# drprojects/superpoint_transformer

Hardware: AMD Instinct MI355X
Metric: Mpoints/s SPT fwd+bwd on S3DIS-scale NAG (higher is better)
Workload: dtype f32 (the reference's shipped matmul class - configs/train.yaml:60-61 `float32_matmul_precision: high` = TF32 / bf16x3 next to `precision: 32` - as bf16x3: matrix products on the bf16 pipe with split operands, attention and the backward of the fused layers and of the attention blocks' Linears hi*hi +

## Files before the change

include/spt_hip.h:

```cpp
#ifndef SPT_HIP_H
#define SPT_HIP_H

#include <stddef.h>
#include <stdint.h>

#ifdef __cplusplus
extern "C" {
#endif

typedef void* spt_stream_t;

enum spt_reduce_op {
  SPT_SUM = 0,
  SPT_MEAN = 1,
  SPT_MIN = 2,
  SPT_MAX = 3
};

typedef struct spt_gn_fwd_tables {
  const float* weight;
  const float* mean_scale;
  float eps;
  float* mean;
  float* rstd;
// ... 462 lines not shown
size_t spt_fused_linear_workspace_bytes(int K, int N);
int spt_fused_linear_fwd_f32(const float* x, int64_t r0, int64_t r1, int K, const float* W,
                             int N, const float* pre_am, const float* pre_scale,
                             const float* pre_bias, float pre_slope, float* h, double* total,
                             void* ws, size_t ws_bytes, spt_stream_t stream);
int spt_fused_linear_bwd_f32(const float* gy, const float* h, int64_t r0, int64_t r1, int N,
                             const float* am, const float* scale, const float* bias,
                             float slope, const float* c1, const float* c2, const float* c3,
                             const float* xprev, int K, const float* pre_am,
                             const float* pre_scale, const float* pre_bias, float pre_slope,
                             const float* W, float* gx, float* gW, int accumulate,
                             double* prev_total, void* ws, size_t ws_bytes, spt_stream_t stream);
int spt_fused_linear_pooled_supported(int K, int N);
int spt_fused_linear_pooled_supported_ex(int K, int N, int mode);
#define SPT_FMLP_BWD_REGISTER_STAGED 4
#define SPT_FMLP_H_BF16 8
#define SPT_FMLP_X_BF16 16
int spt_fused_linear_storage_supported(int K, int N);
int spt_fused_linear_bwd_use_dma(int on);
int spt_fused_linear_bwd_route(int K0, int K, int N, int mode);
int spt_fused_linear_fwd_use_x3(int on);
int spt_fused_linear_fwd_ex_f32(const float* x, int64_t r0, int64_t r1, int K, const float* W,
                                int N, const float* pre_am, const float* pre_scale,
                                const float* pre_bias, float pre_slope, float* h, double* total,
                                int mode, void* ws, size_t ws_bytes, spt_stream_t stream);
int spt_fused_linear_bwd_ex_f32(const float* gy, const float* h, int64_t r0, int64_t r1, int N,
                                const float* am, const float* scale, const float* bias,
                                float slope, const float* c1, const float* c2, const float* c3,
                                const float* xprev, int K, const float* pre_am,
                                const float* pre_scale, const float* pre_bias, float pre_slope,
                                const float* W, float* gx, float* gW, int accumulate,
                                double* prev_total, int mode, void* ws, size_t ws_bytes,
                                spt_stream_t stream);
int spt_fused_linear_bwd_pooled_ex_f32(
    const float* gout, const int32_t* arg, const int32_t* perm, const int32_t* pos_seg,
    const float* h, int64_t p0, int64_t p1, int N, const float* am, const float* scale,
    const float* bias, float slope, const float* c1, const float* c2, const float* c3,
    const float* xprev, int K, const float* pre_am, const float* pre_scale, const float* pre_bias,
    float pre_slope, const float* W, float* gx, float* gW, int accumulate, double* prev_total,
    int mode, void* ws, size_t ws_bytes, spt_stream_t stream);
int spt_fused_linear_bwd_pooled_f32(
    const float* gout, const int32_t* arg, const int32_t* perm, const int32_t* pos_seg,
    const float* h, int64_t p0, int64_t p1, int N, const float* am, const float* scale,
    const float* bias, float slope, const float* c1, const float* c2, const float* c3,
    const float* xprev, int K, const float* pre_am, const float* pre_scale, const float* pre_bias,
    float pre_slope, const float* W, float* gx, float* gW, int accumulate, double* prev_total,
    void* ws, size_t ws_bytes, spt_stream_t stream);

int spt_fused_linear_fwd_runs_f32(const float* x, int nruns, const int64_t* run_r0,
                                  const int64_t* run_r1, const int32_t* run_graph, int num_graphs,
                                  int K, const float* W, int N, const float* pre_am,
                                  const float* pre_scale, const float* pre_bias, float pre_slope,
                                  float* h, double* total, int mode, void* ws, size_t ws_bytes,
                                  spt_stream_t stream);
int spt_fused_linear_bwd_runs_f32(
    const float* gy, const float* h, int nruns, const int64_t* run_r0, const int64_t* run_r1,
    const int32_t* run_graph, int num_graphs, int N, const float* am, const float* scale,
    const float* bias, float slope, const float* c1, const float* c2, const float* c3,
    const float* xprev, int K, const float* pre_am, const float* pre_scale, const float* pre_bias,
    float pre_slope, const float* W, float* gx, float* gW, double* prev_total, int mode, void* ws,
    size_t ws_bytes, spt_stream_t stream);
int spt_fused_linear_bwd_pooled_runs_f32(
    const float* gout, const int32_t* arg, const int32_t* perm, const int32_t* pos_seg,
    const float* h, int nruns, const int64_t* run_p0, const int64_t* run_p1,
    const int32_t* run_graph, int num_graphs, int N, const float* am, const float* scale,
    const float* bias, float slope, const float* c1, const float* c2, const float* c3,
    const float* xprev, int K, const float* pre_am, const float* pre_scale, const float* pre_bias,
    float pre_slope, const float* W, float* gx, float* gW, double* prev_total, int mode, void* ws,
    size_t ws_bytes, spt_stream_t stream);
int spt_fused_linear_fwd_runs_gn_f32(const float* x, int nruns, const int64_t* run_r0,
                                     const int64_t* run_r1, const int32_t* run_graph, int num_graphs,
                                     int K, const float* W, int N, const float* pre_am,
                                     const float* pre_scale, const float* pre_bias, float pre_slope,
                                     float* h, double* total, int mode, void* ws, size_t ws_bytes,
                                     const spt_gn_fwd_tables* norm, spt_stream_t stream);
int spt_fused_linear_bwd_runs_gn_f32(
    const float* gy, const float* h, int nruns, const int64_t* run_r0, const int64_t* run_r1,
    const int32_t* run_graph, int num_graphs, int N, const float* am, const float* scale,
    const float* bias, float slope, const float* c1, const float* c2, const float* c3,
    const float* xprev, int K, const float* pre_am, const float* pre_scale, const float* pre_bias,
    float pre_slope, const float* W, float* gx, float* gW, double* prev_total, int mode, void* ws,
    size_t ws_bytes, const spt_gn_bwd_tables* prev_norm, spt_stream_t stream);
int spt_fused_linear_bwd_fold_supported(int K0, int K, int N, int mode);
int spt_fused_linear_bwd_runs_gn_fold_f32(
    const float* gy, const float* h, int nruns, const int64_t* run_r0, const int64_t* run_r1,
    const int32_t* run_graph, int num_graphs, int N, const float* am, const float* scale,
    const float* bias, float slope, const float* c1, const float* c2, const float* c3,
    const float* xprev, int K, const float* pre_am, const float* pre_scale, const float* pre_bias,
    float pre_slope, const float* W, float* gW, int mode, void* ws, size_t ws_bytes,
    const spt_gn_bwd_tables* prev_norm, const float* x0, int K0, const float* W0, float* gW0,
    spt_stream_t stream);
int spt_fused_linear_bwd_pooled_runs_gn_f32(
    const float* gout, const int32_t* arg, const int32_t* perm, const int32_t* pos_seg,
    const float* h, int nruns, const int64_t* run_p0, const int64_t* run_p1,
    const int32_t* run_graph, int num_graphs, int N, const float* am, const float* scale,
    const float* bias, float slope, const float* c1, const float* c2, const float* c3,
    const float* xprev, int K, const float* pre_am, const float* pre_scale, const float* pre_bias,
    float pre_slope, const float* W, float* gx, float* gW, double* prev_total, int mode, void* ws,
    size_t ws_bytes, const spt_gn_bwd_tables* prev_norm, spt_stream_t stream);

int spt_csr_check_i64(const int64_t* idx, const int64_t* points, const int64_t* pointers, int64_t n,
                      int64_t num_seg, int check_ascending, int32_t* flag, spt_stream_t stream);
int spt_csr_adopt_i64(const int64_t* idx, const int64_t* points, const int64_t* pointers, int64_t n,
                      int64_t num_seg, int32_t* perm32, int32_t* rowptr32, int32_t* flag,
                      spt_stream_t stream);

int spt_fused_linear_pool_supported(int K, int N, int mode);
size_t spt_fused_linear_pool_gram_len(int K);
size_t spt_fused_linear_pool_workspace_bytes(int K, int N);
int spt_fused_linear_fwd_pool_runs_f32(
    const void* x, const int32_t* perm, const int32_t* pos_seg, const int32_t* rowptr,
    const int64_t* seg_graph, int64_t num_seg, int64_t n_rows, int nruns, const int64_t* run_p0,
    const int64_t* run_p1, const int32_t* run_graph, int num_graphs, int K, const float* W, int N,
    const float* gn_weight, const float* gn_bias, const float* gn_mean_scale, float eps, float slope,
    const float* pre_am, const float* pre_scale, const float* pre_bias, float pre_slope, float* out,
    int32_t* arg, int32_t* argpos, float* raw, double* gram, double* total, float* mean, float* rstd,
    float* am, float* scale, int mode, void* ws, size_t ws_bytes, spt_stream_t stream);
int spt_fused_linear_bwd_pool_runs_f32(
    const float* gout, const float* raw, const int32_t* argpos, const int32_t* perm,
    const int32_t* pos_seg, const int64_t* seg_graph, int64_t num_seg, int nruns,
    const int64_t* run_p0, const int64_t* run_p1, const int32_t* run_graph, int num_graphs, int N,
    const float* am, const float* scale, const float* bias, float slope, const float* c1,
    const float* c2, const float* c3, const void* xprev, int K, const float* pre_am,
    const float* pre_scale, const float* pre_bias, float pre_slope, const float* W,
    const double* gram, float* gm, float* gx, float* gW, double* prev_total, int mode, void* ws,
    size_t ws_bytes, spt_stream_t stream);
int spt_fused_linear_bwd_pool_runs_gn_f32(
    const float* gout, const float* raw, const int32_t* argpos, const int32_t* perm,
    const int32_t* pos_seg, const int64_t* seg_graph, int64_t num_seg, int nruns,
    const int64_t* run_p0, const int64_t* run_p1, const int32_t* run_graph, int num_graphs, int N,
    const float* am, const float* scale, const float* bias, float slope, const float* c1,
    const float* c2, const float* c3, const void* xprev, int K, const float* pre_am,
    const float* pre_scale, const float* pre_bias, float pre_slope, const float* W,
    const double* gram, float* gm, float* gx, float* gW, double* prev_total, int mode, void* ws,
    size_t ws_bytes, const spt_gn_bwd_tables* prev_norm, spt_stream_t stream);

size_t spt_cross_entropy_workspace_bytes(int64_t rows);
int spt_cross_entropy_fwd_f32(const float* logits, const int64_t* target, int64_t rows, int C,
                              int64_t ignore_index, float* lse, float* loss, float* count,
                              void* ws, size_t ws_bytes, spt_stream_t stream);
int spt_cross_entropy_bwd_f32(const float* logits, const int64_t* target, const float* lse,
                              int64_t rows, int C, int64_t ignore_index, const float* gout,
                              const float* count, float* glogits, spt_stream_t stream);

int spt_hist_loss_fwd_f32(const float* logits, const int64_t* target, int64_t rows, int C, int ncols,
                          int mode, int64_t ignore_index, const float* weight, float* loss,
                          double* den, int64_t* confmat, void* ws, size_t ws_bytes,
                          spt_stream_t stream);
int spt_hist_loss_bwd_f32(const float* logits, const int64_t* target, int64_t rows, int C, int ncols,
                          int mode, int64_t ignore_index, const float* weight, const float* gout,
                          const double* den, float* glogits, spt_stream_t stream);
size_t spt_edge_affinity_loss_workspace_bytes(int64_t E);
int spt_edge_affinity_loss_fwd_f32(const float* logits, const float* target,
                                   const int64_t* edge_index, int64_t E, const uint8_t* node_void,
                                   const int64_t* node_obj, const int64_t* node_y, int64_t N,
                                   const float* case_weight, const float* pos_weight, float* loss,
                                   double* den, int64_t* stats, int32_t* status, void* ws,
                                   size_t ws_bytes, spt_stream_t stream);
int spt_edge_affinity_loss_bwd_f32(const float* logits, const float* target,
                                   const int64_t* edge_index, int64_t E, const uint8_t* node_void,
                                   const int64_t* node_obj, const int64_t* node_y, int64_t N,
                                   const float* case_weight, const float* pos_weight,
                                   const float* gout, const double* den, float* glogits,
                                   spt_stream_t stream);
int spt_confusion_matrix_i64(const int64_t* pred, const int64_t* target, int64_t rows, int C,
                             int ncols, int64_t* confmat, spt_stream_t stream);
// ... 87 lines not shown
```

superpoint_transformer_amd/_lib.py:

```python
import ctypes
import os

import torch

_HERE = os.path.dirname(os.path.abspath(__file__))
LIB_PATH = os.path.join(_HERE, "lib", "libspt_hip.so")

_c = ctypes
_i64 = _c.c_int64
_int = _c.c_int
_p = _c.c_void_p
_sz = _c.c_size_t
_f32 = _c.c_float
_f64 = _c.c_double

SIGNATURES = {
    "spt_version": (_int, []),
    "spt_last_error": (_c.c_char_p, []),
    "spt_csr_build_workspace_bytes": (_sz, [_i64, _i64]),
    "spt_csr_build": (_int, [_p, _i64, _i64, _p, _p, _p, _sz, _p]),
    "spt_csr_pos_seg": (_int, [_p, _i64, _i64, _p, _p]),
    "spt_csr_gather_i64_i32": (_int, [_p, _p, _i64, _p, _p]),
    "spt_segcsr_reduce_f32": (_int, [_int, _p, _p, _p, _i64, _i64, _int, _p, _p, _p]),
    "spt_segcsr_max_affine_f32": (_int, [_p, _p, _p, _i64, _i64, _int, _p, _p, _p, _f32, _p, _p, _p, _p]),
# ... 44 lines not shown
                                        _p, _p, _p, _p, _p, _p, _int, _f32, _p, _p, _p, _int, _p]),
    "spt_attn_resolve_mode": (_int, [_int]),
    "spt_edge_attn_bwd_route": (_int, [_i64, _i64, _int, _int, _int, _int, _int, _int, _sz]),
    "spt_edge_attn_bwd_ex_workspace_bytes": (_sz, [_i64, _i64, _int, _int, _int, _int]),
    "spt_edge_attn_bwd_el_supported": (_int, [_int, _int, _int, _int, _int]),
    "spt_attn_pack_tile_ids": (_int, [_p, _p, _p, _i64, _p, _p]),
    "spt_edge_attn_bwd_ex_f32": (_int, [_p, _i64, _int, _int, _int, _p, _p, _p, _p, _p, _p, _p, _i64, _p, _int,
                                        _p, _p, _p, _p, _p, _p, _int, _f32, _p, _p, _p, _p,
                                        _p, _p, _int, _p, _p, _p, _p, _p, _p, _int, _p, _sz, _p]),
    "spt_grid_knn_workspace_bytes": (_sz, [_i64, _i64]),
    "spt_knn_use_cell_path": (_int, [_int]),
    "spt_segcsr_use_stream": (_int, [_int]),
    "spt_segcsr_reduce_ex_f32": (_int, [_int, _p, _p, _p, _i64, _i64, _int, _p, _p, _int, _p]),
    "spt_segcsr_max_affine_ex_f32": (_int, [_p, _p, _p, _i64, _i64, _int, _p, _p, _p, _f32, _p, _p, _p,
                                            _int, _p]),
    "spt_grid_knn_ex_f32": (_int, [_p, _i64, _p, _i64, _int, _f32, _f32, _p, _p, _int, _int, _int,
                                   _p, _p, _p, _int, _p, _sz, _p]),
    "spt_grid_knn_geof_f32": (_int, [_p, _i64, _int, _f32, _f32, _p, _p, _int, _int, _int, _int,
                                     _p, _p, _p, _p, _int, _p, _sz, _p]),
    "spt_grid_knn_after_f32": (_int, [_p, _i64, _p, _i64, _int, _f32, _f32, _p, _p, _int, _int, _p, _p,
                                      _p, _p, _p, _sz, _p]),
    "spt_grid_knn_f32": (_int, [_p, _i64, _p, _i64, _int, _f32, _f32, _p, _p, _int, _int, _int,
                                _p, _p, _p, _p, _sz, _p]),
    "spt_point_geof_dense_f32": (_int, [_p, _i64, _p, _int, _int, _int, _int, _p, _p, _p]),
    "spt_point_geof_dense_ld_f32": (_int, [_p, _i64, _p, _int, _i64, _int, _int, _int, _p, _p, _p]),
    "spt_bbox_f32": (_int, [_p, _i64, _p, _p]),
    "spt_knn_subsample_f32": (_int, [_p, _i64, _p, _f32, _int, _p, _p, _p]),
    "spt_grid_cell_ids_f32": (_int, [_p, _i64, _f32, _p, _p, _p, _p]),
    "spt_grid_count_cells_workspace_bytes": (_sz, [_i64]),
    "spt_grid_count_cells_f32": (_int, [_p, _i64, _f32, _p, _p, _p, _p, _sz, _p]),
    "spt_spatial_order_workspace_bytes": (_sz, [_i64, _i64]),
    "spt_spatial_order": (_int, [_p, _i64, _f32, _p, _p, _p, _p, _sz, _p]),
    "spt_point_geof_csr_f32": (_int, [_p, _i64, _p, _p, _int, _int, _int, _p, _p]),
    "spt_vertical_edge_features_f32": (_int, [_p, _i64] + [_p] * 13 + [_p]),
    "spt_edge_affinity_features_f32": (_int, [_p, _i64, _int, _p, _p, _i64, _p, _p]),
    "spt_edge_affinity_features_bwd_f32": (_int, [_p, _p, _i64, _int, _p, _p, _i64, _p, _p]),
    "spt_scatter_pca_f32": (_int, [_p, _p, _p, _i64, _p, _p, _p]),
    "spt_neighbors_dense_to_csr_workspace_bytes": (_sz, [_i64]),
    "spt_neighbors_dense_to_csr": (_int, [_p, _i64, _int, _p, _p, _p, _p, _sz, _p]),
    "spt_horizontal_edge_features_f32": (_int, [_p, _i64, _i64, _p, _p, _p, _p, _p, _p, _p, _int,
                                                _p, _p, _p]),
    "spt_graphnorm_tables_f32": (_int, [_p, _int, _int, _p, _p, _f32, _p, _p, _p, _p, _p]),
    "spt_graphnorm_apply_f32": (_int, [_p, _p, _i64, _int, _int, _p, _p, _p, _f32, _p, _p]),
    "spt_graphnorm_bwd_stats_f32": (_int, [_p, _p, _p, _i64, _int, _int, _p, _p, _p, _f32, _p,
                                           _p, _sz, _p]),
    "spt_graphnorm_bwd_stats_sparse_workspace_bytes": (_sz, [_i64, _int, _int]),
    "spt_graphnorm_bwd_stats_sparse_f32": (_int, [_p, _p, _p, _p, _p, _i64, _i64, _int, _int, _p, _p,
                                                   _p, _f32, _p, _p, _sz, _p]),
    "spt_graphnorm_bwd_tables_f32": (_int, [_p, _int, _int, _p, _p, _p, _p, _p, _p, _p, _p, _p,
                                            _p, _p]),
    "spt_fused_linear_supported": (_int, [_int, _int]),
    "spt_fused_linear_use_split_bf16": (_int, [_int]),
    "spt_fused_linear_bwd_use_dma": (_int, [_int]),
    "spt_fused_linear_bwd_route": (_int, [_int, _int, _int, _int]),
    "spt_fused_linear_fwd_use_x3": (_int, [_int]),
    "spt_fused_linear_pooled_supported": (_int, [_int, _int]),
    "spt_fused_linear_bwd_pooled_f32": (_int, [_p, _p, _p, _p, _p, _i64, _i64, _int, _p, _p, _p, _f32,
                                               _p, _p, _p, _p, _int, _p, _p, _p, _f32, _p, _p, _p,
                                               _int, _p, _p, _sz, _p]),
    "spt_fused_linear_pooled_supported_ex": (_int, [_int, _int, _int]),
    "spt_fused_linear_fwd_ex_f32": (_int, [_p, _i64, _i64, _int, _p, _int, _p, _p, _p, _f32, _p, _p,
                                           _int, _p, _sz, _p]),
    "spt_fused_linear_bwd_ex_f32": (_int, [_p, _p, _i64, _i64, _int, _p, _p, _p, _f32, _p, _p, _p,
                                           _p, _int, _p, _p, _p, _f32, _p, _p, _p, _int, _p, _int, _p,
                                           _sz, _p]),
    "spt_fused_linear_bwd_pooled_ex_f32": (_int, [_p, _p, _p, _p, _p, _i64, _i64, _int, _p, _p, _p, _f32,
                                                  _p, _p, _p, _p, _int, _p, _p, _p, _f32, _p, _p, _p,
                                                  _int, _p, _int, _p, _sz, _p]),
    "spt_fused_linear_workspace_bytes": (_sz, [_int, _int]),
    "spt_fused_linear_fwd_runs_f32": (_int, [_p, _int, _p, _p, _p, _int, _int, _p, _int, _p, _p, _p,
                                             _f32, _p, _p, _int, _p, _sz, _p]),
    "spt_fused_linear_bwd_runs_f32": (_int, [_p, _p, _int, _p, _p, _p, _int, _int, _p, _p, _p, _f32,
                                             _p, _p, _p, _p, _int, _p, _p, _p, _f32, _p, _p, _p, _p,
                                             _int, _p, _sz, _p]),
    "spt_fused_linear_bwd_pooled_runs_f32": (_int, [_p, _p, _p, _p, _p, _int, _p, _p, _p, _int, _int,
                                                    _p, _p, _p, _f32, _p, _p, _p, _p, _int, _p, _p,
                                                    _p, _f32, _p, _p, _p, _p, _int, _p, _sz, _p]),
    "spt_fused_linear_fwd_runs_gn_f32": (_int, [_p, _int, _p, _p, _p, _int, _int, _p, _int, _p, _p, _p,
                                                _f32, _p, _p, _int, _p, _sz, _p, _p]),
    "spt_fused_linear_bwd_runs_gn_f32": (_int, [_p, _p, _int, _p, _p, _p, _int, _int, _p, _p, _p, _f32,
                                                _p, _p, _p, _p, _int, _p, _p, _p, _f32, _p, _p, _p, _p,
                                                _int, _p, _sz, _p, _p]),
    "spt_fused_linear_bwd_fold_supported": (_int, [_int, _int, _int, _int]),
    "spt_fused_linear_bwd_runs_gn_fold_f32": (_int, [_p, _p, _int, _p, _p, _p, _int, _int, _p, _p, _p, _f32,
                                                     _p, _p, _p, _p, _int, _p, _p, _p, _f32, _p, _p,
                                                     _int, _p, _sz, _p, _p, _int, _p, _p, _p]),
    "spt_fused_linear_bwd_pooled_runs_gn_f32": (_int, [_p, _p, _p, _p, _p, _int, _p, _p, _p, _int, _int,
                                                       _p, _p, _p, _f32, _p, _p, _p, _p, _int, _p, _p,
                                                       _p, _f32, _p, _p, _p, _p, _int, _p, _sz, _p, _p]),
    "spt_fused_linear_bwd_pool_runs_gn_f32": (_int, [_p, _p, _p, _p, _p, _p, _i64, _int, _p, _p, _p, _int,
                                                     _int, _p, _p, _p, _f32, _p, _p, _p, _p, _int, _p, _p,
                                                     _p, _f32, _p, _p, _p, _p, _p, _p, _int, _p, _sz, _p, _p]),
    "spt_csr_check_i64": (_int, [_p, _p, _p, _i64, _i64, _int, _p, _p]),
    "spt_csr_adopt_i64": (_int, [_p, _p, _p, _i64, _i64, _p, _p, _p, _p]),
    "spt_fused_linear_pool_supported": (_int, [_int, _int, _int]),
    "spt_fused_linear_pool_gram_len": (_sz, [_int]),
    "spt_fused_linear_pool_workspace_bytes": (_sz, [_int, _int]),
    "spt_fused_linear_fwd_pool_runs_f32": (_int, [_p, _p, _p, _p, _p, _i64, _i64, _int, _p, _p, _p, _int,
                                                  _int, _p, _int, _p, _p, _p, _f32, _f32, _p, _p, _p,
                                                  _f32, _p, _p, _p, _p, _p, _p, _p, _p, _p, _p, _int, _p,
                                                  _sz, _p]),
    "spt_fused_linear_bwd_pool_runs_f32": (_int, [_p, _p, _p, _p, _p, _p, _i64, _int, _p, _p, _p, _int,
                                                  _int, _p, _p, _p, _f32, _p, _p, _p, _p, _int, _p, _p,
                                                  _p, _f32, _p, _p, _p, _p, _p, _p, _int, _p, _sz, _p]),
    "spt_fused_linear_fwd_f32": (_int, [_p, _i64, _i64, _int, _p, _int, _p, _p, _p, _f32, _p, _p,
                                        _p, _sz, _p]),
    "spt_fused_linear_bwd_f32": (_int, [_p, _p, _i64, _i64, _int, _p, _p, _p, _f32, _p, _p, _p,
                                        _p, _int, _p, _p, _p, _f32, _p, _p, _p, _int, _p, _p,
                                        _sz, _p]),
    "spt_unit_sphere_norm_f32": (_int, [_p, _p, _p, _p, _p, _p, _i64, _i64, _p, _p, _p, _p]),
    "spt_unit_sphere_assemble_f32": (_int, [_p, _p, _p, _p, _p, _p, _i64, _i64, _p, _int, _p, _p, _p, _p]),
    "spt_unit_sphere_workspace_bytes": (_sz, [_i64, _i64]),
    "spt_unit_sphere_norm_ws_f32": (_int, [_p, _p, _p, _p, _p, _p, _i64, _i64, _p, _p, _p, _p, _sz, _p]),
    "spt_unit_sphere_assemble_ws_f32": (_int, [_p, _p, _p, _p, _p, _p, _i64, _i64, _p, _int, _p, _p, _p,
                                               _p, _sz, _p]),
    "spt_sparse_sample_workspace_bytes": (_sz, [_i64, _i64]),
    "spt_sparse_sample": (_int, [_p, _i64, _i64, _p, _int, _int, _c.c_uint64, _p, _p, _p, _sz, _p]),
    "spt_segment_std_f32": (_int, [_p, _p, _p, _i64, _int, _p, _p]),
    "spt_segment_mean_orientation_f32": (_int, [_p, _p, _p, _i64, _p, _p]),
    "spt_cluster_graph_edges_workspace_bytes": (_sz, [_i64, _int]),
    "spt_cluster_graph_edges": (_int, [_p, _p, _p, _i64, _int, _f32, _int, _p, _p, _p, _p, _sz, _p]),
    "spt_skinny_linear_supported": (_int, [_int, _int]),
    "spt_narrow_linear_bwd_supported": (_int, [_int, _int]),
    "spt_narrow_linear_bwd_workspace_bytes": (_sz, [_int, _int]),
    "spt_narrow_linear_bwd_f32": (_int, [_p, _p, _p, _i64, _int, _int, _p, _p, _p, _p, _sz, _p]),
    "spt_cross_entropy_workspace_bytes": (_sz, [_i64]),
    "spt_cross_entropy_fwd_f32": (_int, [_p, _p, _i64, _int, _i64, _p, _p, _p, _p, _sz, _p]),
    "spt_cross_entropy_bwd_f32": (_int, [_p, _p, _p, _i64, _int, _i64, _p, _p, _p, _p]),
    "spt_hist_loss_fwd_f32": (_int, [_p, _p, _i64, _int, _int, _int, _i64, _p, _p, _p, _p, _p, _sz, _p]),
    "spt_hist_loss_bwd_f32": (_int, [_p, _p, _i64, _int, _int, _int, _i64, _p, _p, _p, _p, _p]),
    "spt_confusion_matrix_i64": (_int, [_p, _p, _i64, _int, _int, _p, _p]),
    "spt_skinny_dw_supported": (_int, [_int, _int]),
    "spt_skinny_dw_workspace_bytes": (_sz, [_int, _int]),
    "spt_skinny_dw_f32": (_int, [_p, _p, _i64, _int, _int, _p, _p, _p, _sz, _p]),
    "spt_skinny_linear_f32": (_int, [_p, _i64, _int, _p, _p, _int, _p, _p]),
    "spt_skinny_linear_wt_f32": (_int, [_p, _i64, _int, _p, _int, _p, _p]),
    "spt_skinny_pre_supported": (_int, [_int, _int, _int]),
    "spt_skinny_linear_pre_f32": (_int, [_p, _i64, _int, _p, _p, _int, _p, _p, _p, _p, _p, _int, _p, _p]),
    "spt_skinny_dw_pre_f32": (_int, [_p, _p, _i64, _int, _int, _p, _p, _p, _p, _p, _p, _int, _p, _sz, _p]),
    "spt_skinny_use_split_bf16": (_int, [_int]),
    "spt_skinny_linear_pre_m_f32": (_int, [_p, _i64, _int, _p, _p, _int, _p, _p, _p, _p, _p, _int, _p, _int, _p]),
    "spt_skinny_linear_wt_m_f32": (_int, [_p, _i64, _int, _p, _int, _p, _int, _p]),
    "spt_skinny_dw_pre_m_f32": (_int, [_p, _p, _i64, _int, _int, _p, _p, _p, _p, _p, _p, _int, _int, _p, _sz, _p]),
    "spt_skinny_linear_bwd_supported": (_int, [_int, _int, _int, _int]),
    "spt_skinny_linear_bwd_workspace_bytes": (_sz, [_int, _int]),
    "spt_skinny_linear_bwd_m_f32": (_int, [_p, _p, _p, _i64, _int, _int, _p, _p, _p, _p, _p, _p, _p, _int, _int,
                                           _p, _sz, _p]),
    "spt_skinny_bwd_fused": (_int, [_int]),
    "spt_index_inverse": (_int, [_p, _i64, _i64, _p, _p]),
    "spt_select_edges_workspace_bytes": (_sz, [_i64]),
    "spt_select_edges": (_int, [_p, _i64, _i64, _p, _i64, _p, _i64, _p, _p, _p, _sz, _p]),
    "spt_cluster_select_workspace_bytes": (_sz, [_i64, _i64, _i64]),
    "spt_cluster_select": (_int, [_p, _p, _i64, _p, _i64, _i64, _p, _p, _p, _p, _p, _p, _sz, _p]),
    "spt_relabel_consecutive_workspace_bytes": (_sz, [_i64]),
    "spt_relabel_consecutive": (_int, [_p, _p, _i64, _i64, _p, _p, _p, _p, _sz, _p]),
    "spt_radius_ball_workspace_bytes": (_sz, [_i64]),
    "spt_radius_ball_f32": (_int, [_p, _i64, _p, _f32, _int, _p, _i64, _p, _p, _p, _sz, _p]),
    "spt_cluster_pair_anchors_f32": (_int, [_p, _p, _p, _p, _p, _i64, _i64, _int, _int, _p, _p, _p]),
    "spt_adjacency_stats_workspace_bytes": (_sz, [_i64]),
    "spt_adjacency_stats": (_int, [_p, _p, _i64, _i64, _int, _p, _p, _p, _sz, _p]),
    "spt_adjacency_regression": (_int, [_p, _p, _p, _i64, _i64, _int, _f32, _f32, _p, _p, _sz, _p]),
    "spt_adjacency_count_workspace_bytes": (_sz, [_i64]),
    "spt_adjacency_count": (_int, [_p, _i64, _i64, _int, _p, _p, _p, _i64, _int, _p, _p, _p, _sz, _p]),
    "spt_adjacency_fill_workspace_bytes": (_sz, [_i64, _i64]),
    "spt_adjacency_fill": (_int, [_p, _p, _i64, _i64, _int, _f32, _f32, _p, _p, _p, _p, _i64, _int, _int,
                                  _p, _p, _i64, _p, _p, _p, _p, _sz, _p]),
# ... 101 lines not shown
```

superpoint_transformer_amd/csrc/fused_mlp.hip:

```cpp
#include <math.h>
#include <stdlib.h>

#include "common.hpp"

namespace spt {
namespace fmlp {

typedef float f32x4 __attribute__((ext_vector_type(4)));
constexpr int WAVES = 4;
constexpr int TR = 16;
constexpr int MAX_BLOCKS = 1024;
constexpr int MAX_BWD_WAVES = 4096;

__device__ __forceinline__ double xg_sum_d(double v) {
  v += __shfl_xor(v, 16, 64);
  v += __shfl_xor(v, 32, 64);
  return v;
}
__device__ __forceinline__ void wave_sync_lds() {
  __builtin_amdgcn_fence(__ATOMIC_RELEASE, "wavefront");
  __builtin_amdgcn_wave_barrier();
  __builtin_amdgcn_fence(__ATOMIC_ACQUIRE, "wavefront");
}

// ... 563 lines not shown
#pragma unroll
      for (int nb = 0; nb < NBK; ++nb) C[nb] = mfma3_32<LO>(ah, alo, Bh[nb][ks], Bl[nb][ks], C[nb]);
    }
    if constexpr (OUT16) {
      constexpr int ROWB = 2 * N + 16;
      static_assert(TR * ROWB <= TR * LDA * 4, "the packed output tile fits the A-tile buffer");
      static_assert((TR * N / 8) % 64 == 0 || TR * N / 8 < 64, "whole 16-byte chunks");
      wave_sync_lds();
      char* ob = reinterpret_cast<char*>(al);
#pragma unroll
      for (int r = 0; r < 4; ++r) {
        const int rr = 4 * g + r;
#pragma unroll
        for (int nb = 0; nb < NBK; ++nb) {
          const unsigned mine = bf16_bits(C[nb][r]);
          const float vr = __uint_as_float(mine << 16);
          if (rr < cnt) {
            s1[nb] += (double)vr;
            s2[nb] += (double)vr * (double)vr;
          }
          const unsigned other = (unsigned)__builtin_amdgcn_update_dpp(0, (int)mine, 0xB1, 0xF, 0xF, false);
          if ((c & 1) == (r & 1)) {
            const unsigned w = (c & 1) ? (other | (mine << 16)) : (mine | (other << 16));
            *reinterpret_cast<unsigned*>(ob + rr * ROWB + (16 * nb + (c & ~1)) * 2) = w;
          }
        }
      }
      wave_sync_lds();
      constexpr int CPR = N / 8;
      uint16_t* h16 = reinterpret_cast<uint16_t*>(h);
#pragma unroll
      for (int q = lane; q < TR * CPR; q += 64) {
        const int rr = q / CPR, ch = q - rr * CPR;
        if (rr < cnt)
          *reinterpret_cast<uint4*>(h16 + (row0 + rr) * N + ch * 8) =
              *reinterpret_cast<const uint4*>(ob + rr * ROWB + ch * 16);
      }
    } else {
#pragma unroll
      for (int r = 0; r < 4; ++r) {
        const int rr = 4 * g + r;
        if (rr < cnt) {
          float* hr = h + (row0 + rr) * N + c;
#pragma unroll
          for (int nb = 0; nb < NBK; ++nb) {
            const float v = C[nb][r];
            hr[16 * nb] = v;
            s1[nb] += (double)v;
            s2[nb] += (double)v * (double)v;
          }
        }
      }
    }
  }
#pragma unroll
  for (int nb = 0; nb < NBK; ++nb) {
    const double a = xg_sum_d(s1[nb]), b = xg_sum_d(s2[nb]);
    if (g == 0) {
      red[wid][nb * 16 + c] = a;
      red[wid][N + nb * 16 + c] = b;
    }
  }
  __syncthreads();
  double* out = partial + (size_t)blockIdx.x * (2 * N + 1);
  for (int i = threadIdx.x; i < 2 * N; i += WAVES * 64)
    out[i] = ((red[0][i] + red[1][i]) + red[2][i]) + red[3][i];
  if (threadIdx.x == 0) out[2 * N] = (blockIdx.x == 0) ? (double)(r1 - r0) : 0.0;
}

constexpr int WAVES_X3 = 8;
template <int NV, typename V>
__device__ __forceinline__ void split3_bf16(const float (&x)[NV], V& h, V& m, V& l) {
#pragma unroll
  for (int i = 0; i < NV; ++i) {
    const __bf16 a = (__bf16)x[i];
    const float r1 = x[i] - (float)a;
    const __bf16 b = (__bf16)r1;
    const float r2 = r1 - (float)b;
    h[i] = a;
    m[i] = b;
    l[i] = (__bf16)r2;
  }
}
template <int K4, int NBK>
__global__ __launch_bounds__(WAVES_X3 * 64, 2) void fwd_kernel_x3(
    const float* __restrict__ x, int64_t r0, int64_t r1, int K, const float* __restrict__ W,
    const float* __restrict__ am, const float* __restrict__ sc, const float* __restrict__ bs,
    float slope, float* __restrict__ h, double* __restrict__ partial, FmlpRuns rt) {
  constexpr int KP = K4 * 4, KS = (KP + 31) / 32, KP32 = KS * 32, LDA = KP32 + 4, N = NBK * 16;
  constexpr int LDW = KP32 + 8;
  SPT_FMLP_RUN_FWD(N)
  __shared__ __attribute__((aligned(16))) float a_lds[WAVES_X3][TR * LDA];
  __shared__ __attribute__((aligned(16))) float tab[3 * KP32];
  __shared__ __attribute__((aligned(16))) __bf16 wpl[3][N * LDW];
  __shared__ double red[WAVES_X3][2 * N];
  const int lane = threadIdx.x & 63;
  const int wid = __builtin_amdgcn_readfirstlane(threadIdx.x >> 6);
  const int g = lane >> 4, c = lane & 15;
  float* al = a_lds[wid];
  const bool pre = am != nullptr;
  load_table(tab, am, K, KP32);
  load_table(tab + KP32, sc, K, KP32);
  load_table(tab + 2 * KP32, bs, K, KP32);
  for (int i = lane; i < TR * LDA; i += 64) al[i] = 0.f;
  for (int i = threadIdx.x; i < N * KP32; i += WAVES_X3 * 64) {
    const int n = i / KP32, k = i - n * KP32;
    const float w1[1] = {(k < K) ? W[(size_t)n * K + k] : 0.f};
    __bf16 a[1], b[1], cc[1];
    split3_bf16<1>(w1, a, b, cc);
    wpl[0][n * LDW + k] = a[0];
    wpl[1][n * LDW + k] = b[0];
    wpl[2][n * LDW + k] = cc[0];
  }
  __syncthreads();

  double s1[NBK], s2[NBK];
#pragma unroll
  for (int nb = 0; nb < NBK; ++nb) s1[nb] = s2[nb] = 0.0;

  const int64_t ntiles = (r1 - r0 + TR - 1) / TR;
  const int64_t wave = (int64_t)blockIdx.x * WAVES_X3 + wid;
  const int64_t nwaves = (int64_t)gridDim.x * WAVES_X3;
  constexpr int CHP = KP / 4, NITP = (TR * CHP + 63) / 64;
  const bool pref = (K & 3) == 0 && K == KP;
  float4 pv[NITP];
  auto prefetch = [&](int64_t t) {
    const int64_t row0 = r0 + t * TR;
    const int cnt = (t < ntiles) ? (int)((r1 - row0) < TR ? (r1 - row0) : TR) : 0;
#pragma unroll
    for (int j = 0; j < NITP; ++j) {
      const int q = lane + 64 * j, rr = q / CHP, k = (q - rr * CHP) << 2;
      const bool ok = q < TR * CHP && rr < cnt;
      const float4 v = *reinterpret_cast<const float4*>(x + (ok ? (row0 + rr) * K + k : r0 * K));
      pv[j] = ok ? v : make_float4(0.f, 0.f, 0.f, 0.f);
    }
  };
  if (pref && wave < ntiles) prefetch(wave);
  for (int64_t t = wave; t < ntiles; t += nwaves) {
    const int64_t row0 = r0 + t * TR;
    const int cnt = (int)((r1 - row0) < TR ? (r1 - row0) : TR);
    wave_sync_lds();
    if (pref) {
#pragma unroll
      for (int j = 0; j < NITP; ++j) {
        const int q = lane + 64 * j, rr = q / CHP, k = (q - rr * CHP) << 2;
        if (q < TR * CHP) {
          float4 w = pv[j];
          if (pre && rr < cnt) {
            const float4 a = *reinterpret_cast<const float4*>(tab + k);
            const float4 s4 = *reinterpret_cast<const float4*>(tab + KP32 + k);
            const float4 b = *reinterpret_cast<const float4*>(tab + 2 * KP32 + k);
            w.x = fmaf(w.x - a.x, s4.x, b.x); w.y = fmaf(w.y - a.y, s4.y, b.y);
            w.z = fmaf(w.z - a.z, s4.z, b.z); w.w = fmaf(w.w - a.w, s4.w, b.w);
            w.x = w.x > 0.f ? w.x : w.x * slope; w.y = w.y > 0.f ? w.y : w.y * slope;
            w.z = w.z > 0.f ? w.z : w.z * slope; w.w = w.w > 0.f ? w.w : w.w * slope;
          }
          *reinterpret_cast<float4*>(al + rr * LDA + k) = w;
        }
      }
    } else {
      stage_tile<KP32, LDA, KP32>(x, row0, cnt, K, pre, tab, slope, al, nullptr, lane);
    }
    wave_sync_lds();
    if (pref) prefetch(t + nwaves);
    f32x4 C[NBK];
#pragma unroll
    for (int nb = 0; nb < NBK; ++nb) C[nb] = (f32x4){0.f, 0.f, 0.f, 0.f};
#pragma unroll
    for (int ks = 0; ks < KS; ++ks) {
      const float4 a0 = *reinterpret_cast<const float4*>(al + c * LDA + 32 * ks + 8 * g);
      const float4 a1 = *reinterpret_cast<const float4*>(al + c * LDA + 32 * ks + 8 * g + 4);
      const float av[8] = {a0.x, a0.y, a0.z, a0.w, a1.x, a1.y, a1.z, a1.w};
      bf16x8 x1, x2, x3;
      split3_bf16<8>(av, x1, x2, x3);
#pragma unroll
      for (int nb = 0; nb < NBK; ++nb) {
        const int wo = (16 * nb + c) * LDW + 32 * ks + 8 * g;
        const bf16x8 w1 = *reinterpret_cast<const bf16x8*>(&wpl[0][wo]);
        const bf16x8 w2 = *reinterpret_cast<const bf16x8*>(&wpl[1][wo]);
        const bf16x8 w3 = *reinterpret_cast<const bf16x8*>(&wpl[2][wo]);
        f32x4 acc = C[nb];
        acc = __builtin_amdgcn_mfma_f32_16x16x32_bf16(x3, w1, acc, 0, 0, 0);
        acc = __builtin_amdgcn_mfma_f32_16x16x32_bf16(x1, w3, acc, 0, 0, 0);
        acc = __builtin_amdgcn_mfma_f32_16x16x32_bf16(x2, w2, acc, 0, 0, 0);
        acc = __builtin_amdgcn_mfma_f32_16x16x32_bf16(x2, w1, acc, 0, 0, 0);
        acc = __builtin_amdgcn_mfma_f32_16x16x32_bf16(x1, w2, acc, 0, 0, 0);
        acc = __builtin_amdgcn_mfma_f32_16x16x32_bf16(x1, w1, acc, 0, 0, 0);
        C[nb] = acc;
      }
    }
#pragma unroll
    for (int r = 0; r < 4; ++r) {
      const int rr = 4 * g + r;
      if (rr < cnt) {
        float* hr = h + (row0 + rr) * N + c;
#pragma unroll
        for (int nb = 0; nb < NBK; ++nb) {
          const float v = C[nb][r];
          hr[16 * nb] = v;
          s1[nb] += (double)v;
          s2[nb] += (double)v * (double)v;
        }
      }
    }
  }
#pragma unroll
  for (int nb = 0; nb < NBK; ++nb) {
    const double a = xg_sum_d(s1[nb]), b = xg_sum_d(s2[nb]);
    if (g == 0) {
      red[wid][nb * 16 + c] = a;
      red[wid][N + nb * 16 + c] = b;
    }
  }
  __syncthreads();
  double* out = partial + (size_t)blockIdx.x * (2 * N + 1);
  for (int i = threadIdx.x; i < 2 * N; i += WAVES_X3 * 64) {
    double t2 = 0.0;
#pragma unroll
    for (int w = 0; w < WAVES_X3; ++w) t2 += red[w][i];
    out[i] = t2;
  }
  if (threadIdx.x == 0) out[2 * N] = (blockIdx.x == 0) ? (double)(r1 - r0) : 0.0;
}

__host__ __device__ constexpr bool fmlp_bf_wg_reduce(int K4, int NBK, int NW) {
  return NBK * 16 <= NW * TR && K4 > 0;
}
constexpr int fold_zp(int K0) { return (K0 + 16) / 16 * 16; }
constexpr int FOLD_SHIFT_LD = 32;
template <int K4, int NBK, bool NEED_GX, int NW, bool LO, bool POOLED = false, bool PIPE = false,
          bool H16 = false, bool X16 = false, int FK0 = 0>
__global__ __launch_bounds__(NW * 64, NW / 4) void bwd_kernel_bf(
    const float* __restrict__ gy, const float* __restrict__ h, int64_t r0, int64_t r1,
    const float* __restrict__ am, const float* __restrict__ sc, const float* __restrict__ bs,
    float slope, const float* __restrict__ c1, const float* __restrict__ c2,
    const float* __restrict__ c3, const float* __restrict__ xprev, int K,
    const float* __restrict__ pam, const float* __restrict__ psc, const float* __restrict__ pbs,
    float pslope, const float* __restrict__ W, float* __restrict__ gx,
    float* __restrict__ gw_partial, double* __restrict__ pstat_partial, FmlpRuns rt,
    const int32_t* __restrict__ perm = nullptr, const int32_t* __restrict__ pos_seg = nullptr,
    const float* __restrict__ gout = nullptr, const int32_t* __restrict__ arg = nullptr,
    const float* __restrict__ x0 = nullptr, const float* __restrict__ fshift = nullptr,
    float* __restrict__ fold_partial = nullptr) {
  constexpr int KP = K4 * 4, KB = (KP + 15) / 16, KPP = KB * 16, N = NBK * 16;
  constexpr int NS = (N + 31) / 32, NP32 = NS * 32;
  constexpr int LDG = NP32 + 4, LDX = KPP + 4, LDT = NP32 + 8;
  constexpr bool WGR = fmlp_bf_wg_reduce(K4, NBK, NW);
  constexpr bool FOLD = FK0 > 0;
  constexpr int ZP = fold_zp(FOLD ? FK0 : 1), ZB = ZP / 16, LDZ = ZP + 4, FLN = (KPP + ZP) * ZP;
  static_assert(!FOLD || (WGR && NEED_GX && !POOLED && !PIPE && !H16 && !X16 && KP == KPP && ZP <= 32),
                "the fold: dense f32 rows, one table per workgroup");
  static_assert(!FOLD || FLN <= NW * TR * LDX, "the fold table fits the x tile buffers");
  SPT_FMLP_RUN_BWD_T(N, NW, (WGR ? 1 : NW))
  if constexpr (FOLD) {
    if (rt.n > 0) {
      fshift += (size_t)rt.g[blockIdx.y] * FOLD_SHIFT_LD;
      fold_partial += (size_t)blockIdx.y * gridDim.x * FLN;
    }
  }
  __shared__ __attribute__((aligned(16))) float z_lds[FOLD ? NW : 1][FOLD ? TR * LDZ : 4];
  __shared__ float fsh[32];
  __shared__ __attribute__((aligned(16))) float g_lds[NW][TR * LDG];
  __shared__ __attribute__((aligned(16))) float x_lds[NW][TR * LDX];
  __shared__ __attribute__((aligned(16))) __bf16 wt_hi[NEED_GX ? KPP * LDT : 8];
  __shared__ __attribute__((aligned(16))) __bf16 wt_lo[NEED_GX ? KPP * LDT : 8];
  __shared__ __attribute__((aligned(16))) float gt[6 * N];
  __shared__ __attribute__((aligned(16))) float pt[3 * KPP];
  const int lane = threadIdx.x & 63;
  const int wid = __builtin_amdgcn_readfirstlane(threadIdx.x >> 6);
  const int g = lane >> 4, c = lane & 15;
  float* gl = g_lds[wid];
  float* xl = x_lds[wid];
  const bool pre = pam != nullptr;
  if constexpr (NEED_GX) {
    for (int i = threadIdx.x; i < KPP * NP32; i += NW * 64) {
      const int k = i / NP32, n = i - k * NP32;
      const float w = (k < K && n < N) ? W[(size_t)n * K + k] : 0.f;
      const __bf16 hh = (__bf16)w;
      wt_hi[k * LDT + n] = hh;
      wt_lo[k * LDT + n] = (__bf16)(w - (float)hh);
    }
  }
  load_table(gt, am, N, N);
  load_table(gt + N, sc, N, N);
  load_table(gt + 2 * N, bs, N, N);
  load_table(gt + 3 * N, c1, N, N);
  load_table(gt + 4 * N, c2, N, N);
  load_table(gt + 5 * N, c3, N, N);
  load_table(pt, pam, K, KPP);
  load_table(pt + KPP, psc, K, KPP);
  load_table(pt + 2 * KPP, pbs, K, KPP);
  for (int i = lane; i < TR * LDX; i += 64) xl[i] = 0.f;
  for (int i = lane; i < TR * LDG; i += 64) gl[i] = 0.f;
  if constexpr (FOLD) {
    if (threadIdx.x < 32) fsh[threadIdx.x] = (int)threadIdx.x < FK0 ? fshift[threadIdx.x] : 0.f;
  }
  float* zl = z_lds[FOLD ? wid : 0];
  __syncthreads();

  f32x4 FA[FOLD ? KB : 1][ZB], FG[FOLD ? ZB : 1][ZB];
#pragma unroll
  for (int zb = 0; zb < ZB; ++zb) {
#pragma unroll
    for (int kb = 0; kb < (FOLD ? KB : 1); ++kb) FA[kb][zb] = (f32x4){0.f, 0.f, 0.f, 0.f};
#pragma unroll
// ... 678 lines not shown
    for (int j = 0; j < POST_GB; ++j) {
      if (j >= nb) break;
      const int b = b0 + j;
      const double A = s[3 * j], GO = s[3 * j + 1], cnt = s[3 * j + 2];
      if (prev_total) {
        double* tr = prev_total + (size_t)b * len;
        if (cv) {
          tr[c] = A;
          tr[K + c] = GO;
        }
        if (bx == 0 && cl == 0) tr[2 * K] = cnt;
      }
      if (!cv) continue;
      double n = cnt;
      if (n < 1.0) n = 1.0;
      const double sd = (double)pn.rstd[b * K + c], mu = (double)pn.mean[b * K + c];
      const double k2 = w * sd * sd * sd * GO / n;
      const double sumdo = w * sd * A - k2 * n * mu * (1.0 - a);
      pn.c1[b * K + c] = (float)(w * sd);
      pn.c2[b * K + c] = (float)k2;
      pn.c3[b * K + c] = (float)(a * sumdo / n);
      gw += sd * GO;
      gb += A;
      ga += -mu * sumdo;
    }
  }
  if (slice == 0 && cv) {
    pn.gweight[c] = (float)gw;
    pn.gbias[c] = (float)gb;
    pn.gmean_scale[c] = (float)ga;
  }
}

static void bwd_post_launch(const float* gwp, int ntab_w, int NK, float* gW, int accumulate,
                            const double* pst, const FmlpGroups& grp, int K, int B,
                            double* prev_total, const spt_gn_bwd_tables* pn, hipStream_t stream,
                            const FmlpFold* fold = nullptr) {
  const int nA = (NK + 15) / 16;
  spt_gn_bwd_tables none = {};
  int nB = 0;
  if (pn && pn->c1) nB = (K + 15) / 16;
  else if (prev_total) nB = ((2 * K + 1 + 15) / 16) * B;
  FmlpFold fd = {};
  int nF = 0;
  if (fold) {
    fd = *fold;
    fd.first = nA + nB;
    nF = ((K + 15) / 16) * fd.K0;
  }
  bwd_post_kernel<<<nA + nB + nF, 1024, 0, stream>>>(gwp, ntab_w, NK, gW, accumulate, nA, pst, grp, K, B,
                                                     prev_total, (pn && pn->c1) ? *pn : none, fd);
}

static int grid_for_nw(int64_t rows, int per_cu, int nwv) {
  const int64_t tiles = (rows + TR - 1) / TR;
  int64_t blocks = (tiles + nwv - 1) / nwv;
  const int64_t cap = 256 * per_cu;
  if (blocks > cap) blocks = cap;
  if (blocks < 1) blocks = 1;
  return (int)blocks;
}

static int grid_for(int64_t rows, int per_cu) {
  const int64_t tiles = (rows + TR - 1) / TR;
  int64_t blocks = (tiles + WAVES - 1) / WAVES;
  const int64_t cap = 256 * per_cu;
  if (blocks > cap) blocks = cap;
  if (blocks < 1) blocks = 1;
  return (int)blocks;
}

}

bool fmlp_dma_supported(int K, int N);
int fmlp_dma_bwd_launch(bool pooled, bool lo, const float* gy, const float* h, FmlpRuns rt,
                        int64_t max_rows, int N, const float* am, const float* sc, const float* bs,
                        float slope, const float* c1, const float* c2, const float* c3,
                        const float* xprev, int K, const float* pam, const float* psc,
                        const float* pbs, float pslope, const float* W, float* gx,
                        float* gw_partial, double* pstat_partial, const int32_t* perm,
                        const int32_t* pos_seg, const float* gout, const int32_t* arg,
                        hipStream_t stream, bool s16 = false, int* gw_tabs = nullptr,
                        const float* x0 = nullptr, const float* fshift = nullptr,
                        float* fold_partial = nullptr, int K0 = 0, int blocks32 = 0);
bool fmlp_dma_fold_supported(int K0, int K, int N);
bool fmlp_dma_dense_only(int K, int N);
int fmlp_fold_len(int K, int K0);
}

using namespace spt;
using namespace spt::fmlp;

#define SPT_FMLP_SHAPES(X) X(3, 2) X(5, 2) X(8, 2) X(8, 4) X(16, 4) X(16, 8) X(17, 4) X(33, 4)

static std::atomic<int> g_fmlp_mode{1};
static inline int fmlp_mode_of(int mode) { return mode < 0 ? (int)g_fmlp_mode : (mode & 3); }
static std::atomic<int> g_fmlp_x3{[] { const char* e = getenv("SPT_FMLP_X3"); return e ? (atoi(e) != 0) : 1; }()};
extern "C" int spt_fused_linear_fwd_use_x3(int on) {
  const int prev = g_fmlp_x3;
  if (on >= 0) g_fmlp_x3 = on != 0;
  return prev;
}
static std::atomic<int> g_fmlp_dma{1};
static inline bool fmlp_dma_of(int mode) { return g_fmlp_dma != 0 && !(mode >= 0 && (mode & 4)); }
extern "C" int spt_fused_linear_bwd_use_dma(int on) {
  const int prev = g_fmlp_dma;
  if (on >= 0) g_fmlp_dma = on != 0;
  return prev;
}
extern "C" int spt_fused_linear_use_split_bf16(int mode) {
  const int prev = g_fmlp_mode;
  g_fmlp_mode = mode < 0 ? 0 : (mode > 3 ? 3 : mode);
  return prev;
}

#define SPT_FMLP_POOLED_SHAPES(X) X(16, 8) X(16, 4) X(8, 4)
extern "C" int spt_fused_linear_pooled_supported(int K, int N) {
  return spt_fused_linear_pooled_supported_ex(K, N, -1);
}
extern "C" int spt_fused_linear_pooled_supported_ex(int K, int N, int mode) {
  const int k4 = (K + 3) / 4, nbk = N / 16;
  if (N % 16 || fmlp_mode_of(mode) < 1) return 0;
#define X(a, b) if (k4 == a && nbk == b) return 1;
  SPT_FMLP_POOLED_SHAPES(X)
#undef X
  return 0;
}

#define SPT_FMLP_ST_SHAPES(X) X(3, 2) X(8, 4) X(16, 8) X(16, 4)
#define SPT_FMLP_ST_POOLED_SHAPES(X) X(16, 8) X(16, 4) X(8, 4)
extern "C" int spt_fused_linear_storage_supported(int K, int N) {
  const int k4 = (K + 3) / 4, nbk = N / 16;
  if (N % 16) return 0;
#define X(a, b) if (k4 == a && nbk == b) return 1;
  SPT_FMLP_ST_SHAPES(X)
#undef X
  return 0;
}

extern "C" int spt_fused_linear_supported(int K, int N) {
  const int k4 = (K + 3) / 4, nbk = N / 16;
  if (N % 16) return 0;
#define X(a, b) if (k4 == a && nbk == b) return 1;
  SPT_FMLP_SHAPES(X)
#undef X
  return 0;
}

extern "C" size_t spt_fused_linear_workspace_bytes(int K, int N) {
  const size_t fwd = (size_t)MAX_BLOCKS * (2 * N + 1) * 8;
  const size_t bwd = (size_t)MAX_BWD_WAVES * ((size_t)N * K * 4 + (2 * K + 1) * 8);
  return align_up(fwd > bwd ? fwd : bwd, 256) + 4096;
}

static const char* fmlp_make_runs(int nruns, const int64_t* r0, const int64_t* r1, const int32_t* g,
                                  int num_graphs, FmlpRuns* rt, int64_t* max_rows) {
  if (nruns < 1 || nruns > FMLP_MAX_RUNS) return "1 <= nruns <= 16";
  if (num_graphs < 1 || num_graphs > FMLP_MAX_RUNS) return "1 <= num_graphs <= 16";
  if (!r0 || !r1 || !g) return "null run table";
  rt->n = nruns;
  *max_rows = 0;
  for (int r = 0; r < nruns; ++r) {
    if (r1[r] < r0[r] || g[r] < 0 || g[r] >= num_graphs) return "bad run";
    if (r && g[r] < g[r - 1]) return "runs must be sorted by graph";
    rt->r0[r] = r0[r];
    rt->r1[r] = r1[r];
    rt->g[r] = g[r];
    if (r1[r] - r0[r] > *max_rows) *max_rows = r1[r] - r0[r];
  }
  return nullptr;
}
static FmlpGroups fmlp_groups(const FmlpRuns& rt, int num_graphs, int per_run) {
  FmlpGroups grp;
  for (int b = 0; b < FMLP_MAX_RUNS; ++b) grp.start[b] = grp.count[b] = 0;
  for (int r = 0; r < rt.n; ++r) {
    const int b = rt.g[r];
    if (grp.count[b] == 0) grp.start[b] = r * per_run;
    grp.count[b] += per_run;
  }
  (void)num_graphs;
  return grp;
}

static int fmlp_fwd_impl(const char* fn, const float* x, const FmlpRuns& rt, int64_t max_rows,
                         int num_graphs, int K, const float* W, int N, const float* pre_am,
                         const float* pre_scale, const float* pre_bias, float pre_slope, float* h,
                         double* total, int mode, void* ws, size_t ws_bytes, hipStream_t stream,
                         const spt_gn_fwd_tables* norm = nullptr) {
  const int g_fmlp_mode = fmlp_mode_of(mode);
  (void)fn;
  SPT_CHECK_ARG(K >= 1 && N >= 16, "bad shape");
  SPT_CHECK_ARG(spt_fused_linear_supported(K, N), "(K, N) not built");
  SPT_CHECK_ARG(x && W && h && (total || norm) && ws, "null pointer");
  SPT_CHECK_ARG(!norm || (norm->weight && norm->mean_scale && norm->mean && norm->rstd && norm->am &&
                          norm->scale), "incomplete norm tables");
  auto post = [&](const double* partial_, int gx__) {
    if (norm)
      fwd_post_kernel<<<dim3((N + 15) / 16, num_graphs), 1024, 0, stream>>>(
          partial_, fmlp_groups(rt, num_graphs, gx__), N, total, *norm);
    else
      reduce_tables_groups_kernel<double><<<dim3((2 * N + 1 + 15) / 16, num_graphs), 1024, 0, stream>>>(
          partial_, fmlp_groups(rt, num_graphs, gx__), 2 * N + 1, total);
  };
  SPT_CHECK_ARG(ws_bytes >= spt_fused_linear_workspace_bytes(K, N), "workspace too small");
  SPT_CHECK_ARG(!pre_am || (pre_scale && pre_bias), "incomplete pre-normalisation tables");
  const int k4 = (K + 3) / 4, nbk = N / 16;
  const int per_cu = (k4 * nbk <= 32) ? 4 : 2;
  int gx_ = grid_for(max_rows, per_cu);
  const int cap = MAX_BLOCKS / rt.n;
  if (gx_ > cap) gx_ = cap;
  const bool x3 = g_fmlp_mode == 1 && g_fmlp_x3 && !(mode >= 0 && (mode & (SPT_FMLP_H_BF16 | SPT_FMLP_X_BF16)));
  if (x3) {
    const int64_t tiles = (max_rows + TR - 1) / TR;
    int64_t blocks = (tiles + WAVES_X3 - 1) / WAVES_X3;
    const int64_t cap8 = 256 * ((k4 * nbk <= 32) ? 2 : 1);
    if (blocks > cap8) blocks = cap8;
    if (blocks > cap) blocks = cap;
    gx_ = (int)(blocks < 1 ? 1 : blocks);
  }
  const dim3 grid((unsigned)gx_, (unsigned)rt.n);
  const dim3 grid8 = grid;
  double* partial = (double*)ws;
  const bool h16 = mode >= 0 && (mode & SPT_FMLP_H_BF16), x16 = mode >= 0 && (mode & SPT_FMLP_X_BF16);
  if (h16 || x16) {
    SPT_CHECK_ARG(g_fmlp_mode == 3 && h16 && spt_fused_linear_storage_supported(K, N) &&
                  (!x16 || K % 32 == 0),
                  "bf16 activation storage: bf16 matrix mode, a built shape, h stored as bf16");
#define XS(a, b)                                                                                   \
  if (k4 == a && nbk == b) {                                                                       \
    if (x16)                                                                                       \
      fwd_kernel_bf<a, b, false, true, true><<<grid, WAVES * 64, 0, stream>>>(                     \
          x, 0, 0, K, W, pre_am, pre_scale, pre_bias, pre_slope, h, partial, rt);                  \
    else                                                                                           \
      fwd_kernel_bf<a, b, false, false, true><<<grid, WAVES * 64, 0, stream>>>(                    \
          x, 0, 0, K, W, pre_am, pre_scale, pre_bias, pre_slope, h, partial, rt);                  \
  }
    SPT_FMLP_ST_SHAPES(XS)
#undef XS
    post(partial, gx_);
    SPT_CHECK_LAUNCH();
    return 0;
  }
#define X(a, b)                                                                        \
  if (k4 == a && nbk == b) {                                                           \
    if (g_fmlp_mode == 3)                                                              \
      fwd_kernel_bf<a, b, false><<<grid, WAVES * 64, 0, stream>>>(x, 0, 0, K, W, pre_am, pre_scale, \
                                                                  pre_bias, pre_slope, h, partial, rt); \
    else if (g_fmlp_mode == 2)                                                         \
      fwd_kernel_bf<a, b, true><<<grid, WAVES * 64, 0, stream>>>(x, 0, 0, K, W, pre_am, pre_scale, \
                                                                 pre_bias, pre_slope, h, partial, rt);  \
    else if (g_fmlp_mode == 1 && g_fmlp_x3)                                            \
      fwd_kernel_x3<a, b><<<grid8, WAVES_X3 * 64, 0, stream>>>(x, 0, 0, K, W, pre_am, pre_scale, \
                                                               pre_bias, pre_slope, h, partial, rt); \
    else                                                                               \
      fwd_kernel<a, b><<<grid, WAVES * 64, 0, stream>>>(x, 0, 0, K, W, pre_am, pre_scale, \
                                                        pre_bias, pre_slope, h, partial, rt);  \
  }
  SPT_FMLP_SHAPES(X)
#undef X
  post(partial, gx_);
  SPT_CHECK_LAUNCH();
  return 0;
}

extern "C" int spt_fused_linear_fwd_f32(const float* x, int64_t r0, int64_t r1, int K,
                                        const float* W, int N, const float* pre_am,
                                        const float* pre_scale, const float* pre_bias,
                                        float pre_slope, float* h, double* total, void* ws,
                                        size_t ws_bytes, spt_stream_t stream_) {
  return spt_fused_linear_fwd_ex_f32(x, r0, r1, K, W, N, pre_am, pre_scale, pre_bias, pre_slope, h,
                                     total, -1, ws, ws_bytes, stream_);
}
extern "C" int spt_fused_linear_fwd_ex_f32(const float* x, int64_t r0, int64_t r1, int K,
                                           const float* W, int N, const float* pre_am,
                                           const float* pre_scale, const float* pre_bias,
                                           float pre_slope, float* h, double* total, int mode,
                                           void* ws, size_t ws_bytes, spt_stream_t stream_) {
  SPT_CHECK_ARG(r1 >= r0, "bad shape");
  FmlpRuns rt;
  rt.n = 1; rt.g[0] = 0; rt.r0[0] = r0; rt.r1[0] = r1;
  return fmlp_fwd_impl(__func__, x, rt, r1 - r0, 1, K, W, N, pre_am, pre_scale, pre_bias, pre_slope,
                       h, total, mode, ws, ws_bytes, (hipStream_t)stream_);
}
extern "C" int spt_fused_linear_fwd_runs_f32(const float* x, int nruns, const int64_t* run_r0,
                                             const int64_t* run_r1, const int32_t* run_graph,
                                             int num_graphs, int K, const float* W, int N,
                                             const float* pre_am, const float* pre_scale,
                                             const float* pre_bias, float pre_slope, float* h,
                                             double* total, int mode, void* ws, size_t ws_bytes,
                                             spt_stream_t stream_) {
  FmlpRuns rt;
  int64_t max_rows;
  const char* err = fmlp_make_runs(nruns, run_r0, run_r1, run_graph, num_graphs, &rt, &max_rows);
  SPT_CHECK_ARG(!err, err ? err : "");
  return fmlp_fwd_impl(__func__, x, rt, max_rows, num_graphs, K, W, N, pre_am, pre_scale, pre_bias,
                       pre_slope, h, total, mode, ws, ws_bytes, (hipStream_t)stream_);
}
extern "C" int spt_fused_linear_fwd_runs_gn_f32(const float* x, int nruns, const int64_t* run_r0,
                                                const int64_t* run_r1, const int32_t* run_graph,
                                                int num_graphs, int K, const float* W, int N,
                                                const float* pre_am, const float* pre_scale,
                                                const float* pre_bias, float pre_slope, float* h,
                                                double* total, int mode, void* ws, size_t ws_bytes,
                                                const spt_gn_fwd_tables* norm, spt_stream_t stream_) {
  FmlpRuns rt;
  int64_t max_rows;
  const char* err = fmlp_make_runs(nruns, run_r0, run_r1, run_graph, num_graphs, &rt, &max_rows);
  SPT_CHECK_ARG(!err, err ? err : "");
  SPT_CHECK_ARG(norm, "null norm descriptor");
  return fmlp_fwd_impl(__func__, x, rt, max_rows, num_graphs, K, W, N, pre_am, pre_scale, pre_bias,
                       pre_slope, h, total, mode, ws, ws_bytes, (hipStream_t)stream_, norm);
}

static int fmlp_bwd_impl(bool pooled, const float* gy, const float* gout, const int32_t* arg,
                         const int32_t* perm, const int32_t* pos_seg, const float* h,
                         const FmlpRuns& rt, int64_t max_rows, int num_graphs, int N,
                         const float* am, const float* scale, const float* bias, float slope,
                         const float* c1, const float* c2, const float* c3, const float* xprev,
                         int K, const float* pre_am, const float* pre_scale, const float* pre_bias,
                         float pre_slope, const float* W, float* gx, float* gW, int accumulate,
                         double* prev_total, int mode, void* ws, size_t ws_bytes,
                         hipStream_t stream, const spt_gn_bwd_tables* prev_norm = nullptr,
                         const float* fold_x0 = nullptr, int fold_K0 = 0, const float* fold_W0 = nullptr,
                         float* fold_gW0 = nullptr) {
  const int g_fmlp_mode = fmlp_mode_of(mode);
  const bool g_fmlp_split_bf16 = g_fmlp_mode >= 1;
  if (fold_x0) {
    SPT_CHECK_ARG(!pooled && !gx && fold_W0 && fold_gW0 && prev_norm && pre_am,
                  "fold: dense layer, no gx, norm tables");
    SPT_CHECK_ARG(spt_fused_linear_bwd_fold_supported(fold_K0, K, N, mode), "fold: shape pair or mode not built");
    SPT_CHECK_ARG(((size_t)fold_x0 & (fold_K0 % 4 == 0 ? 15 : 3)) == 0, "fold: x0 alignment");
  }
  const bool want_prev = prev_total || prev_norm;
  SPT_CHECK_ARG(!prev_norm || (prev_norm->weight && prev_norm->mean_scale && prev_norm->mean &&
                               prev_norm->rstd && prev_norm->c1 && prev_norm->c2 && prev_norm->c3 &&
                               prev_norm->gweight && prev_norm->gbias && prev_norm->gmean_scale),
                "incomplete norm tables");
  SPT_CHECK_ARG(K >= 1 && N >= 16, "bad shape");
  SPT_CHECK_ARG(h && am && scale && bias && c1 && c2 && c3 && xprev && W && gW && ws, "null pointer");
  SPT_CHECK_ARG(ws_bytes >= spt_fused_linear_workspace_bytes(K, N), "workspace too small");
  if (pooled) {
    SPT_CHECK_ARG(spt_fused_linear_pooled_supported_ex(K, N, g_fmlp_mode),
                  "(K, N) has no pooled kernel in this matrix mode");
    SPT_CHECK_ARG(gout && arg && perm && pos_seg && gx, "null pointer");
    SPT_CHECK_ARG(!want_prev || pre_am, "previous-layer statistics need its tables");
  } else {
    SPT_CHECK_ARG(spt_fused_linear_supported(K, N), "(K, N) not built");
    SPT_CHECK_ARG(gy, "null pointer");
    SPT_CHECK_ARG(!want_prev || ((gx || fold_x0) && pre_am), "previous-layer statistics need gx and its tables");
  }
  const int k4 = (K + 3) / 4, nbk = N / 16;
  int gx_ = 1, nwv = 1;
  float* gwp = (float*)ws;
  double* pst = (double*)((char*)ws + align_up((size_t)MAX_BWD_WAVES * N * K * 4, 256));
  double* pstp = want_prev ? pst : nullptr;
  const int nr = rt.n;
  auto cap_grid = [&](int g_, int nw_) {
    const int cap = MAX_BWD_WAVES / (nw_ * nr);
    return g_ > cap ? (cap < 1 ? 1 : cap) : g_;
  };
#define XP(a, b)                                                                                 \
  if (k4 == a && nbk == b) {                                                                     \
     \
     \
    constexpr bool big = (a * b >= 32);                                                          \
    constexpr int NWB = (a * b > 128) ? 4 : (big ? 8 : 4);                                       \
    gx_ = cap_grid(grid_for_nw(max_rows, (a * b > 128) ? 1 : (big ? ((a * b <= 32) ? 2 : 1) : 4), NWB), NWB); \
    nwv = NWB;                                                                                   \
    gw_tabs = gx_ * (fmlp_bf_wg_reduce(a, b, NWB) ? 1 : NWB);                                    \
    const dim3 grid((unsigned)gx_, (unsigned)nr);                                                \
    if (g_fmlp_mode == 3)                                                                        \
      bwd_kernel_bf<a, b, true, NWB, false, true><<<grid, NWB * 64, 0, stream>>>(                \
          nullptr, h, 0, 0, am, scale, bias, slope, c1, c2, c3, xprev, K, pre_am, pre_scale,     \
          pre_bias, pre_slope, W, gx, gwp, pstp, rt, perm, pos_seg, gout, arg);                  \
    else                                                                                         \
      bwd_kernel_bf<a, b, true, NWB, true, true><<<grid, NWB * 64, 0, stream>>>(                 \
          nullptr, h, 0, 0, am, scale, bias, slope, c1, c2, c3, xprev, K, pre_am, pre_scale,     \
          pre_bias, pre_slope, W, gx, gwp, pstp, rt, perm, pos_seg, gout, arg);                  \
  }
#define X(a, b)                                                                                  \
  if (k4 == a && nbk == b) {                                                                     \
    constexpr bool big = (a * b >= 32);                 \
    constexpr int NWV = big ? 8 : 4;                                                             \
             \
                                \
     \
     \
    constexpr int NWB = (a * b > 128) ? 4 : NWV;                                                 \
    if (g_fmlp_split_bf16) {                                                                     \
      gx_ = cap_grid(grid_for_nw(max_rows, (a * b > 128) ? 1 : (big ? ((a * b <= 32) ? 2 : 1) : 4), NWB), NWB); \
      nwv = NWB;                                                                                 \
      gw_tabs = gx_ * (fmlp_bf_wg_reduce(a, b, NWB) ? 1 : NWB);                                  \
    } else {                                                                                     \
      gx_ = cap_grid(grid_for_nw(max_rows, big ? ((a * b <= 32) ? 2 : 1) : 4, NWV), NWV);        \
      nwv = NWV;                                                                                 \
      gw_tabs = gx_ * NWV;                                                                       \
    }                                                                                            \
    const dim3 grid((unsigned)gx_, (unsigned)nr);                                                \
     \
     \
    constexpr bool PIPE_ = (a * b > 128);             \
    if (PIPE_ && K % 4 == 0 && g_fmlp_mode == 3 && gx)                                           \
      bwd_kernel_bf<a, b, true, NWB, false, false, PIPE_><<<grid, NWB * 64, 0, stream>>>(        \
          gy, h, 0, 0, am, scale, bias, slope, c1, c2, c3, xprev, K, pre_am, pre_scale,          \
          pre_bias, pre_slope, W, gx, gwp, pstp, rt);                                            \
    else if (PIPE_ && K % 4 == 0 && g_fmlp_split_bf16 && gx)                                     \
      bwd_kernel_bf<a, b, true, NWB, true, false, PIPE_><<<grid, NWB * 64, 0, stream>>>(         \
          gy, h, 0, 0, am, scale, bias, slope, c1, c2, c3, xprev, K, pre_am, pre_scale,          \
          pre_bias, pre_slope, W, gx, gwp, pstp, rt);                                            \
    else if (g_fmlp_mode == 3 && gx)                                                             \
      bwd_kernel_bf<a, b, true, NWB, false><<<grid, NWB * 64, 0, stream>>>(                      \
          gy, h, 0, 0, am, scale, bias, slope, c1, c2, c3, xprev, K, pre_am, pre_scale,          \
          pre_bias, pre_slope, W, gx, gwp, pstp, rt);                                            \
    else if (g_fmlp_mode == 3)                                                                   \
      bwd_kernel_bf<a, b, false, NWB, false><<<grid, NWB * 64, 0, stream>>>(                     \
          gy, h, 0, 0, am, scale, bias, slope, c1, c2, c3, xprev, K, pre_am, pre_scale,          \
          pre_bias, pre_slope, W, nullptr, gwp, nullptr, rt);                                    \
    else if (g_fmlp_split_bf16 && gx)                                                            \
      bwd_kernel_bf<a, b, true, NWB, true><<<grid, NWB * 64, 0, stream>>>(                       \
          gy, h, 0, 0, am, scale, bias, slope, c1, c2, c3, xprev, K, pre_am, pre_scale,          \
          pre_bias, pre_slope, W, gx, gwp, pstp, rt);                                            \
    else if (g_fmlp_split_bf16)                                                                  \
// ... 6 lines not shown
          pre_bias, pre_slope, W, gx, gwp, pstp, rt);                                            \
    else                                                                                         \
      bwd_kernel<a, b, false, NWV, big><<<grid, NWV * 64, 0, stream>>>(                          \
          gy, h, 0, 0, am, scale, bias, slope, c1, c2, c3, xprev, K, pre_am, pre_scale,          \
          pre_bias, pre_slope, W, nullptr, gwp, nullptr, rt);                                    \
  }
  float* fold_tabs = nullptr;
  float* fold_shift = nullptr;
  const int blocks32 = (K == 32 && N == 32) ? cap_grid(grid_for_nw(max_rows, 4, 4), 4) : 0;
  const bool dma_dense_only = fmlp_dma_dense_only(K, N);
  int per_run = 0;
  int gw_tabs = 0;
  const bool h16 = mode >= 0 && (mode & SPT_FMLP_H_BF16), x16 = mode >= 0 && (mode & SPT_FMLP_X_BF16);
  if (h16 || x16) {
    SPT_CHECK_ARG(g_fmlp_mode == 3 && h16 && spt_fused_linear_storage_supported(K, N) &&
                  (!x16 || K % 16 == 0),
                  "bf16 activation storage: bf16 matrix mode, a built shape, h stored as bf16");
#define XSP(a, b)                                                                                \
  if (pooled && k4 == a && nbk == b) {                                                           \
    constexpr bool big = (a * b >= 32);                                                          \
    constexpr int NWB = (a * b > 128) ? 4 : (big ? 8 : 4);                                       \
    gx_ = cap_grid(grid_for_nw(max_rows, (a * b > 128) ? 1 : (big ? ((a * b <= 32) ? 2 : 1) : 4), NWB), NWB); \
    nwv = NWB;                                                                                   \
    gw_tabs = gx_ * (fmlp_bf_wg_reduce(a, b, NWB) ? 1 : NWB);                                    \
    const dim3 grid((unsigned)gx_, (unsigned)nr);                                                \
    if (x16)                                                                                     \
      bwd_kernel_bf<a, b, true, NWB, false, true, false, true, true><<<grid, NWB * 64, 0, stream>>>( \
          nullptr, h, 0, 0, am, scale, bias, slope, c1, c2, c3, xprev, K, pre_am, pre_scale,     \
          pre_bias, pre_slope, W, gx, gwp, pstp, rt, perm, pos_seg, gout, arg);                  \
    else                                                                                         \
      bwd_kernel_bf<a, b, true, NWB, false, true, false, true, false><<<grid, NWB * 64, 0, stream>>>( \
          nullptr, h, 0, 0, am, scale, bias, slope, c1, c2, c3, xprev, K, pre_am, pre_scale,     \
          pre_bias, pre_slope, W, gx, gwp, pstp, rt, perm, pos_seg, gout, arg);                  \
  }
#define XSD(a, b)                                                                                \
  if (!pooled && k4 == a && nbk == b) {                                                          \
    constexpr bool big = (a * b >= 32);                                                          \
    constexpr int NWV = big ? 8 : 4;                                                             \
    constexpr int NWB = (a * b > 128) ? 4 : NWV;                                                 \
    gx_ = cap_grid(grid_for_nw(max_rows, (a * b > 128) ? 1 : (big ? ((a * b <= 32) ? 2 : 1) : 4), NWB), NWB); \
    nwv = NWB;                                                                                   \
    gw_tabs = gx_ * (fmlp_bf_wg_reduce(a, b, NWB) ? 1 : NWB);                                    \
    const dim3 grid((unsigned)gx_, (unsigned)nr);                                                \
    if (gx && x16)                                                                               \
      bwd_kernel_bf<a, b, true, NWB, false, false, false, true, true><<<grid, NWB * 64, 0, stream>>>( \
          gy, h, 0, 0, am, scale, bias, slope, c1, c2, c3, xprev, K, pre_am, pre_scale,          \
          pre_bias, pre_slope, W, gx, gwp, pstp, rt);                                            \
    else if (gx)                                                                                 \
      bwd_kernel_bf<a, b, true, NWB, false, false, false, true, false><<<grid, NWB * 64, 0, stream>>>( \
          gy, h, 0, 0, am, scale, bias, slope, c1, c2, c3, xprev, K, pre_am, pre_scale,          \
          pre_bias, pre_slope, W, gx, gwp, pstp, rt);                                            \
    else if (x16)                                                                                \
      bwd_kernel_bf<a, b, false, NWB, false, false, false, true, true><<<grid, NWB * 64, 0, stream>>>( \
          gy, h, 0, 0, am, scale, bias, slope, c1, c2, c3, xprev, K, pre_am, pre_scale,          \
          pre_bias, pre_slope, W, nullptr, gwp, nullptr, rt);                                    \
    else                                                                                         \
      bwd_kernel_bf<a, b, false, NWB, false, false, false, true, false><<<grid, NWB * 64, 0, stream>>>( \
          gy, h, 0, 0, am, scale, bias, slope, c1, c2, c3, xprev, K, pre_am, pre_scale,          \
          pre_bias, pre_slope, W, nullptr, gwp, nullptr, rt);                                    \
  }
    if (x16 && gx && fmlp_dma_of(mode) && fmlp_dma_supported(K, N) && !dma_dense_only) {
      per_run = fmlp_dma_bwd_launch(pooled, false, gy, h, rt, max_rows, N, am, scale, bias, slope, c1,
                                    c2, c3, xprev, K, pre_am, pre_scale, pre_bias, pre_slope, W, gx,
                                    gwp, pstp, perm, pos_seg, gout, arg, stream, true, &gw_tabs);
    } else {
      SPT_FMLP_ST_POOLED_SHAPES(XSP)
      SPT_FMLP_ST_SHAPES(XSD)
      per_run = gx_ * nwv;
    }
#undef XSP
#undef XSD
  } else if (fold_x0) {
    constexpr size_t FOLD_MAX_TABS = 1024;
    const int flen = fmlp_fold_len(K, fold_K0);
    SPT_CHECK_ARG((FOLD_MAX_TABS * ((size_t)N * K + flen) + FMLP_MAX_RUNS * FOLD_SHIFT_LD) * 4 <=
                  (size_t)MAX_BWD_WAVES * N * K * 4, "fold: tables do not fit the workspace");
    fold_tabs = gwp + FOLD_MAX_TABS * N * K;
    fold_shift = fold_tabs + FOLD_MAX_TABS * flen;
    fold_shift_kernel<<<num_graphs, 1024, 0, stream>>>(fold_x0, fold_K0, rt, fold_shift);
    if (fmlp_dma_of(mode) && fmlp_dma_fold_supported(fold_K0, K, N)) {
      per_run = fmlp_dma_bwd_launch(false, true, gy, h, rt, max_rows, N, am, scale, bias, slope, c1, c2,
                                    c3, xprev, K, pre_am, pre_scale, pre_bias, pre_slope, W, nullptr,
                                    gwp, pstp, nullptr, nullptr, nullptr, nullptr, stream, false,
                                    &gw_tabs, fold_x0, fold_shift, fold_tabs, fold_K0, blocks32);
    } else if (fold_K0 == 18 && k4 == 8 && nbk == 2) {
      constexpr int NWB = 4;
      gx_ = cap_grid(grid_for_nw(max_rows, 4, NWB), NWB);
      nwv = NWB;
      gw_tabs = gx_;
      const dim3 grid((unsigned)gx_, (unsigned)nr);
      bwd_kernel_bf<8, 2, true, NWB, true, false, false, false, false, 18><<<grid, NWB * 64, 0, stream>>>(
          gy, h, 0, 0, am, scale, bias, slope, c1, c2, c3, xprev, K, pre_am, pre_scale, pre_bias,
          pre_slope, W, nullptr, gwp, pstp, rt, nullptr, nullptr, nullptr, nullptr, fold_x0, fold_shift,
          fold_tabs);
      per_run = gx_ * nwv;
    }
    SPT_CHECK_ARG((size_t)gw_tabs * nr <= FOLD_MAX_TABS, "fold: more tables than the workspace layout holds");
  } else if (g_fmlp_split_bf16 && gx && fmlp_dma_of(mode) && fmlp_dma_supported(K, N) &&
             !(pooled && dma_dense_only)) {
    per_run = fmlp_dma_bwd_launch(pooled, g_fmlp_mode != 3, gy, h, rt, max_rows, N, am, scale, bias,
                                  slope, c1, c2, c3, xprev, K, pre_am, pre_scale, pre_bias, pre_slope,
                                  W, gx, gwp, pstp, perm, pos_seg, gout, arg, stream, false, &gw_tabs,
                                  nullptr, nullptr, nullptr, 0, blocks32);
  } else if (pooled) {
    SPT_FMLP_POOLED_SHAPES(XP)
    per_run = gx_ * nwv;
  } else {
    SPT_FMLP_SHAPES(X)
    per_run = gx_ * nwv;
  }
#undef X
#undef XP
  SPT_CHECK_ARG(per_run > 0, "no kernel for this shape");
  FmlpFold fd = {};
  if (fold_x0) {
    fd.tabs = fold_tabs;
    fd.shift = fold_shift;
    fd.gW0 = fold_gW0;
    fd.W0 = fold_W0;
    fd.am0 = pre_am;
    fd.K0 = fold_K0;
    fd.ZP = fold_zp(fold_K0);
    fd.grp = fmlp_groups(rt, num_graphs, gw_tabs);
  }
  bwd_post_launch(gwp, gw_tabs * nr, N * K, gW, accumulate, pst, fmlp_groups(rt, num_graphs, per_run), K,
                  num_graphs, prev_total, prev_norm, stream, fold_x0 ? &fd : nullptr);
  SPT_CHECK_LAUNCH();
  return 0;
}

extern "C" int spt_fused_linear_bwd_pooled_f32(
    const float* gout, const int32_t* arg, const int32_t* perm, const int32_t* pos_seg,
    const float* h, int64_t p0, int64_t p1, int N, const float* am, const float* scale,
    const float* bias, float slope, const float* c1, const float* c2, const float* c3,
    const float* xprev, int K, const float* pre_am, const float* pre_scale, const float* pre_bias,
    float pre_slope, const float* W, float* gx, float* gW, int accumulate, double* prev_total,
    void* ws, size_t ws_bytes, spt_stream_t stream_) {
  return spt_fused_linear_bwd_pooled_ex_f32(gout, arg, perm, pos_seg, h, p0, p1, N, am, scale, bias,
                                            slope, c1, c2, c3, xprev, K, pre_am, pre_scale, pre_bias,
                                            pre_slope, W, gx, gW, accumulate, prev_total, -1, ws,
                                            ws_bytes, stream_);
}
extern "C" int spt_fused_linear_bwd_pooled_ex_f32(
    const float* gout, const int32_t* arg, const int32_t* perm, const int32_t* pos_seg,
    const float* h, int64_t p0, int64_t p1, int N, const float* am, const float* scale,
    const float* bias, float slope, const float* c1, const float* c2, const float* c3,
    const float* xprev, int K, const float* pre_am, const float* pre_scale, const float* pre_bias,
    float pre_slope, const float* W, float* gx, float* gW, int accumulate, double* prev_total,
    int mode, void* ws, size_t ws_bytes, spt_stream_t stream_) {
  SPT_CHECK_ARG(p1 >= p0, "bad shape");
  FmlpRuns rt;
  rt.n = 1; rt.g[0] = 0; rt.r0[0] = p0; rt.r1[0] = p1;
  return fmlp_bwd_impl(true, nullptr, gout, arg, perm, pos_seg, h, rt, p1 - p0, 1, N, am, scale, bias,
                       slope, c1, c2, c3, xprev, K, pre_am, pre_scale, pre_bias, pre_slope, W, gx, gW,
                       accumulate, prev_total, mode, ws, ws_bytes, (hipStream_t)stream_);
}
extern "C" int spt_fused_linear_bwd_pooled_runs_f32(
    const float* gout, const int32_t* arg, const int32_t* perm, const int32_t* pos_seg,
    const float* h, int nruns, const int64_t* run_p0, const int64_t* run_p1,
    const int32_t* run_graph, int num_graphs, int N, const float* am, const float* scale,
    const float* bias, float slope, const float* c1, const float* c2, const float* c3,
    const float* xprev, int K, const float* pre_am, const float* pre_scale, const float* pre_bias,
    float pre_slope, const float* W, float* gx, float* gW, double* prev_total, int mode, void* ws,
    size_t ws_bytes, spt_stream_t stream_) {
  FmlpRuns rt;
  int64_t max_rows;
  const char* err = fmlp_make_runs(nruns, run_p0, run_p1, run_graph, num_graphs, &rt, &max_rows);
// ... 275 lines not shown
```

superpoint_transformer_amd/csrc/fused_mlp_dma.hip:

```cpp
#include <math.h>

#include "common.hpp"

#ifndef SPT_FDMA_SKIP
#define SPT_FDMA_SKIP 0
#endif

namespace spt {
namespace fdma {

typedef float f32x4 __attribute__((ext_vector_type(4)));
typedef __bf16 bf16x8 __attribute__((ext_vector_type(8)));
typedef __bf16 bf16x4 __attribute__((ext_vector_type(4)));
typedef short s16x4 __attribute__((ext_vector_type(4)));
constexpr int TR = 16;

__device__ __forceinline__ double xg_sum_d(double v) {
  v += __shfl_xor(v, 16, 64);
  v += __shfl_xor(v, 32, 64);
  return v;
}
__device__ __forceinline__ void lds_order() {
  __builtin_amdgcn_fence(__ATOMIC_RELEASE, "wavefront");
  __builtin_amdgcn_wave_barrier();
  __builtin_amdgcn_fence(__ATOMIC_ACQUIRE, "wavefront");
}
__device__ __forceinline__ void lds_dma16(const void* g, float* lds) {
#if SPT_FDMA_SKIP & 32
  return;
#endif
  const unsigned a = __builtin_amdgcn_readfirstlane(
      (unsigned)(size_t)((__attribute__((address_space(3))) void*)lds));
  asm volatile("s_mov_b32 m0, %0\n\ts_nop 0\n\tglobal_load_lds_dwordx4 %1, off"
               :: "s"(a), "v"(g) : "memory");
}
__device__ __forceinline__ void lds_dma4(const void* g, float* lds) {
#if SPT_FDMA_SKIP & 32
  return;
#endif
  const unsigned a = __builtin_amdgcn_readfirstlane(
      (unsigned)(size_t)((__attribute__((address_space(3))) void*)lds));
  asm volatile("s_mov_b32 m0, %0\n\ts_nop 0\n\tglobal_load_lds_dword %1, off"
               :: "s"(a), "v"(g) : "memory");
}
__device__ __forceinline__ void wait_vm0() {
  asm volatile("s_waitcnt vmcnt(0)" ::: "memory");
  __builtin_amdgcn_fence(__ATOMIC_ACQUIRE, "wavefront");
}
__device__ __forceinline__ void wait_lds() {
  asm volatile("s_waitcnt lgkmcnt(0)" ::: "memory");
}
__device__ __forceinline__ int opaque(int v) {
  asm volatile("" : "+v"(v));
  return v;
}
template <int NV, typename V>
__device__ __forceinline__ void split_bf16(const float (&x)[NV], V& hi, V& lo) {
#pragma unroll
  for (int i = 0; i < NV; ++i) {
    const __bf16 h = (__bf16)x[i];
    hi[i] = h;
    lo[i] = (__bf16)(x[i] - (float)h);
  }
}
template <bool LO>
__device__ __forceinline__ f32x4 mfma3_32(const bf16x8& ah, const bf16x8& al, const bf16x8& bh,
                                          const bf16x8& bl, f32x4 c) {
  if constexpr (LO) {
    c = __builtin_amdgcn_mfma_f32_16x16x32_bf16(al, bh, c, 0, 0, 0);
    c = __builtin_amdgcn_mfma_f32_16x16x32_bf16(ah, bl, c, 0, 0, 0);
  }
  return __builtin_amdgcn_mfma_f32_16x16x32_bf16(ah, bh, c, 0, 0, 0);
}
template <bool LO>
__device__ __forceinline__ f32x4 mfma3_16(const bf16x4& ah, const bf16x4& al, const bf16x4& bh,
                                          const bf16x4& bl, f32x4 c) {
  const s16x4 AH = __builtin_bit_cast(s16x4, ah), AL = __builtin_bit_cast(s16x4, al);
  const s16x4 BH = __builtin_bit_cast(s16x4, bh), BL = __builtin_bit_cast(s16x4, bl);
  if constexpr (LO) {
    c = __builtin_amdgcn_mfma_f32_16x16x16bf16_1k(AL, BH, c, 0, 0, 0);
    c = __builtin_amdgcn_mfma_f32_16x16x16bf16_1k(AH, BL, c, 0, 0, 0);
  }
  return __builtin_amdgcn_mfma_f32_16x16x16bf16_1k(AH, BH, c, 0, 0, 0);
}

template <int R>
__device__ __forceinline__ int pick_lane(int v, int base, int sel) {
  int r = __builtin_amdgcn_readlane(v, base);
#pragma unroll
  for (int j = 1; j < R; ++j) r = (sel == j) ? __builtin_amdgcn_readlane(v, base + j) : r;
  return r;
}

constexpr int fold_len(int K, int K0) { return (K + (K0 + 16) / 16 * 16) * ((K0 + 16) / 16 * 16); }
template <int K, int N, int NW, int OCC, bool LO, bool POOLED, bool S16 = false, int FK0 = 0>
__global__ __launch_bounds__(NW * 64, OCC) void bwd_dma_kernel(
    const float* __restrict__ gy, const float* __restrict__ h, int64_t r0, int64_t r1,
    const float* __restrict__ am, const float* __restrict__ sc, const float* __restrict__ bs,
    float slope, const float* __restrict__ c1, const float* __restrict__ c2,
    const float* __restrict__ c3, const float* __restrict__ xprev,
    const float* __restrict__ pam, const float* __restrict__ psc, const float* __restrict__ pbs,
    float pslope, const float* __restrict__ W, float* __restrict__ gx,
    float* __restrict__ gw_partial, double* __restrict__ pstat_partial,
    const int32_t* __restrict__ perm, const int32_t* __restrict__ pos_seg,
    const float* __restrict__ gout, const int32_t* __restrict__ arg, FmlpRuns rt,
    const float* __restrict__ x0 = nullptr, const float* __restrict__ fshift = nullptr,
    float* __restrict__ fold_partial = nullptr) {
  constexpr bool FOLD = FK0 > 0;
  constexpr int FOLD_K0 = FK0;
  static_assert(!FOLD || (!POOLED && !S16), "the fold reads dense f32 rows");
  constexpr int ZP = (FK0 + 16) / 16 * 16, ZB = ZP / 16;
  constexpr bool X0_DMA16 = FK0 % 4 == 0 && TR * FK0 * 4 <= 1024;
  constexpr int X0N = X0_DMA16 ? 1 : (TR * FK0 + 63) / 64;
  constexpr int X0LEN = X0_DMA16 ? 256 : 64 * X0N;
  static_assert(!FOLD || ZP <= 32, "the shift table holds 32 columns");
  constexpr int NC = N / 4, KC = K / 4, NBK = N / 16, KB = K / 16, NS = N / 32;
  if (rt.n > 0) {
    const int run_ = blockIdx.y, gph_ = rt.g[run_];
    r0 = rt.r0[run_];
    r1 = rt.r1[run_];
    am += (size_t)gph_ * N; sc += (size_t)gph_ * N;
    c1 += (size_t)gph_ * N; c2 += (size_t)gph_ * N; c3 += (size_t)gph_ * N;
    if (pam) { pam += (size_t)gph_ * K; psc += (size_t)gph_ * K; }
    gw_partial += (size_t)run_ * gridDim.x * N * K;
    if (pstat_partial) pstat_partial += (size_t)run_ * gridDim.x * NW * (2 * K + 1);
    if constexpr (FOLD) {
      fshift += (size_t)gph_ * 32;
      fold_partial += (size_t)run_ * gridDim.x * fold_len(K, FK0);
    }
  }
  constexpr int HI = TR * NC / 64, XI = TR * KC / 64;
  constexpr int RH = 64 / NC;
  constexpr int NSEG = RH;
  constexpr int LDT = N + 8;
  constexpr int W_H = TR * N, W_X = TR * K, W_G = POOLED ? NSEG * N : 0;
  static_assert(K % 16 == 0 && N % 32 == 0 && (TR * NC) % 64 == 0 && (TR * KC) % 64 == 0, "shape");
  __shared__ __attribute__((aligned(16))) float lw[NW][W_H + W_X + 2 * W_G];
  __shared__ __attribute__((aligned(16))) __bf16 wt_hi[K * LDT];
  __shared__ __attribute__((aligned(16))) __bf16 wt_lo[LO ? K * LDT : 8];
  __shared__ __attribute__((aligned(16))) float pt[3 * K];
  __shared__ __attribute__((aligned(16))) float x0b[FOLD ? NW : 1][FOLD ? X0LEN : 4];
  __shared__ float fsh[32];
  const int lane = threadIdx.x & 63;
  const int wid = __builtin_amdgcn_readfirstlane(threadIdx.x >> 6);
  const int g = lane >> 4, c = lane & 15;
  float* HB = lw[wid];
  float* XB = HB + W_H;
  float* GO = XB + W_X;
  int* AR = reinterpret_cast<int*>(GO + W_G);
  const bool pre = pam != nullptr;
  for (int i = threadIdx.x; i < K * N; i += NW * 64) {
    const int k = i / N, n = i - k * N;
    const float w = W[(size_t)n * K + k];
    const __bf16 hh = (__bf16)w;
    wt_hi[k * LDT + n] = hh;
    if constexpr (LO) wt_lo[k * LDT + n] = (__bf16)(w - (float)hh);
  }
  if constexpr (FOLD) {
    if (threadIdx.x < 32) fsh[threadIdx.x] = threadIdx.x < FOLD_K0 ? fshift[threadIdx.x] : 0.f;
  }
  for (int i = threadIdx.x; i < K; i += NW * 64) {
    pt[i] = pre ? pam[i] : 0.f;
    pt[K + i] = pre ? psc[i] : 1.f;
    pt[2 * K + i] = pre ? pbs[i] : 0.f;
  }
  __syncthreads();

  f32x4 C3[NBK][KB];
#pragma unroll
  for (int nb = 0; nb < NBK; ++nb)
#pragma unroll
    for (int kb = 0; kb < KB; ++kb) C3[nb][kb] = (f32x4){0.f, 0.f, 0.f, 0.f};
  double p1[KB], p2[KB];
#pragma unroll
  for (int kb = 0; kb < KB; ++kb) p1[kb] = p2[kb] = 0.0;
  f32x4 FA[FOLD ? KB : 1][ZB], FG[ZB][ZB];
#pragma unroll
  for (int zb = 0; zb < ZB; ++zb) {
#pragma unroll
    for (int kb = 0; kb < (FOLD ? KB : 1); ++kb) FA[kb][zb] = (f32x4){0.f, 0.f, 0.f, 0.f};
#pragma unroll
    for (int za = 0; za < ZB; ++za) FG[za][zb] = (f32x4){0.f, 0.f, 0.f, 0.f};
  }
  float* X0B = x0b[FOLD ? wid : 0];

  const int64_t ntiles = (r1 - r0 + TR - 1) / TR;
  const int64_t wave = (int64_t)blockIdx.x * NW + wid;
  const int64_t nwaves = (int64_t)gridDim.x * NW;

  const float4 t_am = *reinterpret_cast<const float4*>(am + 4 * (lane % NC));
  const float4 t_sc = *reinterpret_cast<const float4*>(sc + 4 * (lane % NC));
  const float4 t_bs = *reinterpret_cast<const float4*>(bs + 4 * (lane % NC));
  const float4 t_c1 = *reinterpret_cast<const float4*>(c1 + 4 * (lane % NC));
  const float4 t_c2 = *reinterpret_cast<const float4*>(c2 + 4 * (lane % NC));
  const float4 t_c3 = *reinterpret_cast<const float4*>(c3 + 4 * (lane % NC));
  int ln = opaque(lane);
  auto gh1 = [&](float hh, float gg, float aa, float ss, float bb, float q1, float q2, float q3) {
    const float o = hh - aa;
    if (slope != 1.f) {
      const float y = fmaf(o, ss, bb);
      gg = (y > 0.f) ? gg : gg * slope;
    }
    return fmaf(q1, gg, -fmaf(q2, o, q3));
  };
  auto gh_of = [&](const float4& hv, const float4& gv) {
    return make_float4(gh1(hv.x, gv.x, t_am.x, t_sc.x, t_bs.x, t_c1.x, t_c2.x, t_c3.x),
                       gh1(hv.y, gv.y, t_am.y, t_sc.y, t_bs.y, t_c1.y, t_c2.y, t_c3.y),
                       gh1(hv.z, gv.z, t_am.z, t_sc.z, t_bs.z, t_c1.z, t_c2.z, t_c3.z),
                       gh1(hv.w, gv.w, t_am.w, t_sc.w, t_bs.w, t_c1.w, t_c2.w, t_c3.w));
  };
  auto pick = [&](int v, int base) {
    const int hi = ln / NC;
    int r = __builtin_amdgcn_readlane(v, base);
#pragma unroll
    for (int j = 1; j < RH; ++j) r = (hi == j) ? __builtin_amdgcn_readlane(v, base + j) : r;
    return r;
  };
  constexpr int RX = 64 / KC;
  auto pickx = [&](int v, int base) {
    const int hx = ln / KC;
    int r = __builtin_amdgcn_readlane(v, base);
#pragma unroll
    for (int j = 1; j < RX; ++j) r = (hx == j) ? __builtin_amdgcn_readlane(v, base + j) : r;
    return r;
  };

  int rid_n = 0, seg_n = 0;
  auto load_ids = [&](int64_t t) {
    rid_n = seg_n = 0;
    const int64_t rowf = r0 + t * TR;
    if constexpr (POOLED) {
      if (t < ntiles && rowf + lane < r1 && lane < TR) {
        rid_n = perm[rowf + lane];
        seg_n = pos_seg[rowf + lane];
      }
    } else {
      if (t < ntiles && lane < TR) rid_n = (rowf + lane < r1) ? lane : 0;
    }
  };
  constexpr int NC16 = N / 8, RH16 = 64 / NC16, HI16 = TR / RH16;
  constexpr int KC16 = K / 8, RX16 = 64 / KC16, XI16 = (TR + RX16 - 1) / RX16;
  static_assert(!S16 || (TR % RH16 == 0 && RX16 <= TR), "bf16 rows: whole DMA instructions per tile");
  auto issue_h = [&](int64_t t, int rid_l, int seg_l) {
    if (t >= ntiles) return;
    const int64_t row0 = r0 + t * TR;
    const int hi = ln / NC, n4 = ln % NC;
    if constexpr (S16) {
      const uint16_t* hb = reinterpret_cast<const uint16_t*>(h) + (POOLED ? 0 : row0 * N);
      const int h16 = ln / NC16, p16 = ln % NC16;
#pragma unroll
      for (int i = 0; i < HI16; ++i)
        lds_dma16(hb + (int64_t)pick_lane<RH16>(rid_l, RH16 * i, h16) * N + 8 * p16,
                  HB + W_H / 2 + 256 * i);
    } else {
      const float* hb = POOLED ? h : h + row0 * N;
#pragma unroll
      for (int i = 0; i < HI; ++i) {
        const int rr7 = (hi + RH * i) & 7;
        lds_dma16(hb + (int64_t)pick(rid_l, RH * i) * N + 4 * (n4 ^ rr7), HB + 256 * i);
      }
    }
    if constexpr (POOLED) {
      const int cnt = (int)((r1 - row0) < TR ? (r1 - row0) : TR);
      const int s0 = __builtin_amdgcn_readlane(seg_l, 0);
      const int s1 = __builtin_amdgcn_readfirstlane(__shfl(seg_l, cnt - 1, 64));
      const int64_t sgm = (s0 + hi < s1) ? s0 + hi : s1;
      lds_dma16(gout + sgm * N + 4 * n4, GO);
      lds_dma16(arg + sgm * N + 4 * n4, reinterpret_cast<float*>(AR));
    }
  };
  auto issue_x = [&](int64_t t, int rid_l) {
    if (t >= ntiles) return;
    const int64_t row0 = r0 + t * TR;
    if constexpr (FOLD) {
      const int cnt = (int)((r1 - row0) < TR ? (r1 - row0) : TR);
      if constexpr (X0_DMA16) {
        const int last = cnt * FOLD_K0 - 4;
        lds_dma16(x0 + row0 * FOLD_K0 + (4 * ln < last ? 4 * ln : last), X0B);
      } else {
        const int last = cnt * FOLD_K0 - 1;
#pragma unroll
        for (int i = 0; i < X0N; ++i) {
          const int f = 64 * i + ln;
          lds_dma4(x0 + row0 * FOLD_K0 + (f < last ? f : last), X0B + 64 * i);
        }
      }
    }
    if constexpr (S16) {
      const uint16_t* xb = reinterpret_cast<const uint16_t*>(xprev) + (POOLED ? 0 : row0 * K);
      const int x16 = ln / KC16, q16 = ln % KC16;
#pragma unroll
      for (int i = 0; i < XI16; ++i)
        lds_dma16(xb + (int64_t)pick_lane<RX16>(rid_l, RX16 * i, x16) * K + 8 * q16,
                  XB + W_X / 2 + 256 * i);
    } else {
      const float* xb = POOLED ? xprev : xprev + row0 * K;
      const int hx = ln / KC, px = ln % KC;
#pragma unroll
      for (int i = 0; i < XI; ++i) {
        const int rr = hx + RX * i;
        lds_dma16(xb + (int64_t)pickx(rid_l, RX * i) * K + 4 * (px ^ (4 * ((rr >> 2) & 1))), XB + 256 * i);
      }
    }
  };

  load_ids(wave);
  int rid_l = rid_n, seg_l = seg_n;
  issue_h(wave, rid_l, seg_l);
  issue_x(wave, rid_l);
  load_ids(wave + nwaves);
  for (int64_t t = wave; t < ntiles; t += nwaves) {
    const int64_t row0 = r0 + t * TR;
    const int cnt = (int)((r1 - row0) < TR ? (r1 - row0) : TR);
    ln = opaque(ln);
    const int hi = ln / NC, n4 = ln % NC, hx = ln / KC, px = ln % KC, g = ln >> 4, c = ln & 15;
    float4 gyv[POOLED ? 1 : HI];
    if constexpr (!POOLED) {
#pragma unroll
      for (int i = 0; i < HI; ++i) {
        const int rr = hi + RH * i;
        gyv[i] = (rr < cnt) ? *reinterpret_cast<const float4*>(gy + (row0 + rr) * N + 4 * n4)
                            : make_float4(0.f, 0.f, 0.f, 0.f);
      }
    }
    wait_vm0();
    lds_order();
    if constexpr (S16) {
#pragma unroll
      for (int i = 0; i < XI; ++i) {
        const int rr = hx + RX * i;
        const int cx = px ^ (4 * ((rr >> 2) & 1));
        const uint2 u = *reinterpret_cast<const uint2*>(
            reinterpret_cast<const uint16_t*>(XB + W_X / 2) + rr * K + 4 * cx);
        *reinterpret_cast<float4*>(XB + rr * K + 4 * px) =
            make_float4(__uint_as_float(u.x << 16), __uint_as_float(u.x & 0xffff0000u),
                        __uint_as_float(u.y << 16), __uint_as_float(u.y & 0xffff0000u));
      }
    }
    if constexpr (!(SPT_FDMA_SKIP & 1)) {
      const int s0 = POOLED ? __builtin_amdgcn_readlane(seg_l, 0) : 0;
      const int s1 = POOLED ? __builtin_amdgcn_readfirstlane(__shfl(seg_l, cnt - 1, 64)) : 0;
      const bool in_lds = s1 - s0 < NSEG;
#pragma unroll
      for (int i = 0; i < HI; ++i) {
        const int rr = hi + RH * i;
        float* slot = HB + rr * N + 4 * (n4 ^ (rr & 7));
        float4 hv;
        if constexpr (S16) {
          const uint2 u = *reinterpret_cast<const uint2*>(
              reinterpret_cast<const uint16_t*>(HB + W_H / 2) + rr * N + 4 * n4);
          hv = make_float4(__uint_as_float(u.x << 16), __uint_as_float(u.x & 0xffff0000u),
                           __uint_as_float(u.y << 16), __uint_as_float(u.y & 0xffff0000u));
        } else {
          hv = *reinterpret_cast<const float4*>(slot);
        }
        float4 gv;
        if constexpr (POOLED) {
          const int rid = pick(rid_l, RH * i);
          const int sg = pick(seg_l, RH * i);
          int4 av;
          if (in_lds) {
            gv = *reinterpret_cast<const float4*>(GO + (sg - s0) * N + 4 * n4);
            av = *reinterpret_cast<const int4*>(AR + (sg - s0) * N + 4 * n4);
          } else {
            gv = *reinterpret_cast<const float4*>(gout + (int64_t)sg * N + 4 * n4);
            av = *reinterpret_cast<const int4*>(arg + (int64_t)sg * N + 4 * n4);
          }
          gv = make_float4(av.x == rid ? gv.x : 0.f, av.y == rid ? gv.y : 0.f,
                           av.z == rid ? gv.z : 0.f, av.w == rid ? gv.w : 0.f);
        } else {
          gv = gyv[i];
        }
        *reinterpret_cast<float4*>(slot) = gh_of(hv, gv);
      }
      if (cnt < TR) {
#pragma unroll
        for (int i = 0; i < HI; ++i) {
          const int rr = hi + RH * i;
          if (rr >= cnt)
            *reinterpret_cast<float4*>(HB + rr * N + 4 * (n4 ^ (rr & 7))) = make_float4(0.f, 0.f, 0.f, 0.f);
        }
      }
    }
    lds_order();
    if constexpr (!(SPT_FDMA_SKIP & 2)) {
      bf16x4 Xh[KB], Xl[KB];
#pragma unroll
      for (int kb = 0; kb < KB; ++kb) {
        const int k = 16 * kb + c;
        float xv[4];
#pragma unroll
        for (int r = 0; r < 4; ++r) {
          float v = XB[(4 * g + r) * K + 4 * ((4 * kb + (c >> 2)) ^ (4 * (g & 1))) + (c & 3)];
          if (pre) {
            v = fmaf(v - pt[k], pt[K + k], pt[2 * K + k]);
            v = (v > 0.f) ? v : v * pslope;
          }
          xv[r] = v;
        }
        split_bf16<4>(xv, Xh[kb], Xl[kb]);
      }
#pragma unroll
      for (int nb = 0; nb < NBK; ++nb) {
        float gv[4];
#pragma unroll
        for (int r = 0; r < 4; ++r)
          gv[r] = HB[(4 * g + r) * N + 4 * ((4 * nb + (c >> 2)) ^ (4 * (g & 1) + r)) + (c & 3)];
        bf16x4 gh4, gl4;
        split_bf16<4>(gv, gh4, gl4);
#pragma unroll
        for (int kb = 0; kb < KB; ++kb) C3[nb][kb] = mfma3_16<LO>(gh4, gl4, Xh[kb], Xl[kb], C3[nb][kb]);
      }
    }
    f32x4 CX[KB];
#pragma unroll
    for (int kb = 0; kb < KB; ++kb) CX[kb] = (f32x4){0.f, 0.f, 0.f, 0.f};
    if constexpr (!(SPT_FDMA_SKIP & 4)) {
#pragma unroll
      for (int sg = 0; sg < NS; ++sg) {
        const float4 a0 = *reinterpret_cast<const float4*>(HB + c * N + 4 * ((8 * sg + 2 * g) ^ (c & 7)));
        const float4 a1 = *reinterpret_cast<const float4*>(HB + c * N + 4 * ((8 * sg + 2 * g + 1) ^ (c & 7)));
        const float av[8] = {a0.x, a0.y, a0.z, a0.w, a1.x, a1.y, a1.z, a1.w};
        bf16x8 ah, alo;
        split_bf16<8>(av, ah, alo);
#pragma unroll
        for (int kb = 0; kb < KB; ++kb) {
          const bf16x8 bh = *reinterpret_cast<const bf16x8*>(wt_hi + (16 * kb + c) * LDT + 32 * sg + 8 * g);
          bf16x8 bl = bh;
          if constexpr (LO) bl = *reinterpret_cast<const bf16x8*>(wt_lo + (16 * kb + c) * LDT + 32 * sg + 8 * g);
          CX[kb] = mfma3_32<LO>(ah, alo, bh, bl, CX[kb]);
        }
      }
    }
    const int rid_cur = rid_l;
    wait_lds();
    issue_h(t + nwaves, rid_n, seg_n);
    bf16x4 X0h[ZB], X0l[ZB];
    if constexpr (FOLD) {
#pragma unroll
      for (int zb = 0; zb < ZB; ++zb) {
        const int col = 16 * zb + c;
        float x0v[4];
#pragma unroll
        for (int r = 0; r < 4; ++r) {
          const int rr = 4 * g + r;
          const float xr = X0B[rr * FOLD_K0 + (col < FOLD_K0 ? col : 0)];
          const float one = (col == FOLD_K0) ? 1.f : 0.f;
          x0v[r] = (rr < cnt) ? ((col < FOLD_K0) ? xr - fsh[col] : one) : 0.f;
        }
        split_bf16<4>(x0v, X0h[zb], X0l[zb]);
      }
#pragma unroll
      for (int za = 0; za < ZB; ++za)
#pragma unroll
        for (int zb = 0; zb < ZB; ++zb)
          FG[za][zb] = mfma3_16<LO>(X0h[za], X0l[za], X0h[zb], X0l[zb], FG[za][zb]);
    }
#pragma unroll
    for (int kb = 0; kb < KB; ++kb) {
      const int k = 16 * kb + c;
      float ggv[4] = {0.f, 0.f, 0.f, 0.f};
#pragma unroll
      for (int r = 0; r < 4; ++r) {
        float* xs = XB + (4 * g + r) * K + 4 * ((4 * kb + (c >> 2)) ^ (4 * (g & 1))) + (c & 3);
        const float v = CX[kb][r];
        if (!(SPT_FDMA_SKIP & 8) && pre) {
// ... 47 lines not shown
          for (int kb = 0; kb < KB; ++kb)
#pragma unroll
            for (int r = 0; r < 4; ++r) red[(16 * nb + 4 * g + r) * LDR + 16 * kb + c] = C3[nb][kb][r];
      }
      __syncthreads();
      if (wid == 0) {
#pragma unroll
        for (int nb = 0; nb < NBK; ++nb)
#pragma unroll
          for (int kb = 0; kb < KB; ++kb)
#pragma unroll
            for (int r = 0; r < 4; ++r) C3[nb][kb][r] += red[(16 * nb + 4 * g + r) * LDR + 16 * kb + c];
      }
      __syncthreads();
    }
  }
  if (wid == 0) {
    float* gwp = gw_partial + (size_t)blockIdx.x * N * K;
#pragma unroll
    for (int nb = 0; nb < NBK; ++nb)
#pragma unroll
      for (int kb = 0; kb < KB; ++kb)
#pragma unroll
        for (int r = 0; r < 4; ++r)
          gwp[(size_t)(16 * nb + 4 * g + r) * K + 16 * kb + c] = C3[nb][kb][r];
  }
  if constexpr (FOLD) {
    constexpr int FLN = fold_len(K, FK0);
    static_assert(FLN <= NW * (W_H + W_X + 2 * W_G), "the fold table fits the tile buffers");
    float* red = &lw[0][0];
    for (int w = 1; w < NW; ++w) {
      if (wid == w) {
#pragma unroll
        for (int zb = 0; zb < ZB; ++zb)
#pragma unroll
          for (int r = 0; r < 4; ++r) {
#pragma unroll
            for (int kb = 0; kb < KB; ++kb) red[(16 * kb + 4 * g + r) * ZP + 16 * zb + c] = FA[kb][zb][r];
#pragma unroll
            for (int za = 0; za < ZB; ++za) red[(K + 16 * za + 4 * g + r) * ZP + 16 * zb + c] = FG[za][zb][r];
          }
      }
      __syncthreads();
      if (wid == 0) {
#pragma unroll
        for (int zb = 0; zb < ZB; ++zb)
#pragma unroll
          for (int r = 0; r < 4; ++r) {
#pragma unroll
            for (int kb = 0; kb < KB; ++kb) FA[kb][zb][r] += red[(16 * kb + 4 * g + r) * ZP + 16 * zb + c];
#pragma unroll
            for (int za = 0; za < ZB; ++za) FG[za][zb][r] += red[(K + 16 * za + 4 * g + r) * ZP + 16 * zb + c];
          }
      }
      __syncthreads();
    }
    if (wid == 0) {
      float* fp = fold_partial + (size_t)blockIdx.x * FLN;
#pragma unroll
      for (int zb = 0; zb < ZB; ++zb)
#pragma unroll
        for (int r = 0; r < 4; ++r) {
#pragma unroll
          for (int kb = 0; kb < KB; ++kb) fp[(16 * kb + 4 * g + r) * ZP + 16 * zb + c] = FA[kb][zb][r];
#pragma unroll
          for (int za = 0; za < ZB; ++za) fp[(K + 16 * za + 4 * g + r) * ZP + 16 * zb + c] = FG[za][zb][r];
        }
    }
  }
  if (pstat_partial) {
    double* pp = pstat_partial + (size_t)wave * (2 * K + 1);
#pragma unroll
    for (int kb = 0; kb < KB; ++kb) {
      const double a = xg_sum_d(p1[kb]), b = xg_sum_d(p2[kb]);
      if (g == 0) {
        pp[16 * kb + c] = a;
        pp[K + 16 * kb + c] = b;
      }
    }
    if (lane == 0) pp[2 * K] = (wave == 0) ? (double)(r1 - r0) : 0.0;
  }
}

}

bool fmlp_dma_fold_supported(int K0, int K, int N) {
  return (K0 == 12 && K == 32 && N == 64) || (K0 == 18 && K == 32 && N == 32);
}
int fmlp_fold_len(int K, int K0) { return fdma::fold_len(K, K0); }
bool fmlp_dma_supported(int K, int N) {
  return (K == 64 && N == 128) || (K == 32 && N == 64) || (K == 64 && N == 64) || (K == 32 && N == 32);
}
bool fmlp_dma_dense_only(int K, int N) { return K == 32 && N == 32; }

bool fmlp_dma_fold_supported(int K0, int K, int N);
int fmlp_dma_bwd_launch(bool pooled, bool lo, const float* gy, const float* h, FmlpRuns rt,
                        int64_t max_rows, int N, const float* am, const float* sc, const float* bs,
                        float slope, const float* c1, const float* c2, const float* c3,
                        const float* xprev, int K, const float* pam, const float* psc,
                        const float* pbs, float pslope, const float* W, float* gx,
                        float* gw_partial, double* pstat_partial, const int32_t* perm,
                        const int32_t* pos_seg, const float* gout, const int32_t* arg,
                        hipStream_t stream, bool s16, int* gw_tabs, const float* x0,
                        const float* fshift, float* fold_partial, int K0, int blocks32) {
  using namespace fdma;
  const int64_t tiles = (max_rows + TR - 1) / TR;
  const int nr = rt.n < 1 ? 1 : rt.n;
  if (K == 32 && N == 32) {
    if (pooled || s16 || blocks32 < 1) return 0;
    const dim3 grid((unsigned)blocks32, (unsigned)nr);
    if (x0) {
      if (!fmlp_dma_fold_supported(K0, K, N) || !lo || !fshift || !fold_partial || !pam) return 0;
      bwd_dma_kernel<32, 32, 4, 4, true, false, false, 18><<<grid, 4 * 64, 0, stream>>>(
          gy, h, 0, 0, am, sc, bs, slope, c1, c2, c3, xprev, pam, psc, pbs, pslope, W, nullptr,
          gw_partial, pstat_partial, perm, pos_seg, gout, arg, rt, x0, fshift, fold_partial);
    } else if (lo) {
      bwd_dma_kernel<32, 32, 4, 4, true, false><<<grid, 4 * 64, 0, stream>>>(
          gy, h, 0, 0, am, sc, bs, slope, c1, c2, c3, xprev, pam, psc, pbs, pslope, W, gx,
          gw_partial, pstat_partial, perm, pos_seg, gout, arg, rt);
    } else {
      bwd_dma_kernel<32, 32, 4, 4, false, false><<<grid, 4 * 64, 0, stream>>>(
          gy, h, 0, 0, am, sc, bs, slope, c1, c2, c3, xprev, pam, psc, pbs, pslope, W, gx,
          gw_partial, pstat_partial, perm, pos_seg, gout, arg, rt);
    }
    if (gw_tabs) *gw_tabs = blocks32;
    return blocks32 * 4;
  }
  if (x0) {
    if (!fmlp_dma_fold_supported(K0, K, N) || pooled || s16 || !lo || !fshift || !fold_partial || !pam) return 0;
    int64_t blocks = (tiles + 8 - 1) / 8;
    const int64_t cap = (256 * 2) / nr > 1 ? (256 * 2) / nr : 1;
    if (blocks > cap) blocks = cap;
    if (blocks < 1) blocks = 1;
    const dim3 grid((unsigned)blocks, (unsigned)nr);
    bwd_dma_kernel<32, 64, 8, 4, true, false, false, 12><<<grid, 8 * 64, 0, stream>>>(
        gy, h, 0, 0, am, sc, bs, slope, c1, c2, c3, xprev, pam, psc, pbs, pslope, W, nullptr,
        gw_partial, pstat_partial, perm, pos_seg, gout, arg, rt, x0, fshift, fold_partial);
    if (gw_tabs) *gw_tabs = (int)blocks;
    return (int)blocks * 8;
  }
#define SPT_DMA_CASE(KK, NN, NWV, PER_CU, OCC)                                                        \
  if (K == KK && N == NN) {                                                                        \
    int64_t blocks = (tiles + NWV - 1) / NWV;                                                      \
                                      \
    const int64_t cap = (256 * PER_CU) / nr > 1 ? (256 * PER_CU) / nr : 1;                         \
    if (blocks > cap) blocks = cap;                                                                \
    if (blocks < 1) blocks = 1;                                                                    \
    const dim3 grid((unsigned)blocks, (unsigned)nr);                                               \
    if (s16 && pooled)                                                                             \
      bwd_dma_kernel<KK, NN, NWV, OCC, false, true, true><<<grid, NWV * 64, 0, stream>>>(          \
          gy, h, 0, 0, am, sc, bs, slope, c1, c2, c3, xprev, pam, psc, pbs, pslope, W, gx,         \
          gw_partial, pstat_partial, perm, pos_seg, gout, arg, rt);                                \
    else if (s16)                                                                                  \
      bwd_dma_kernel<KK, NN, NWV, OCC, false, false, true><<<grid, NWV * 64, 0, stream>>>(         \
          gy, h, 0, 0, am, sc, bs, slope, c1, c2, c3, xprev, pam, psc, pbs, pslope, W, gx,         \
          gw_partial, pstat_partial, perm, pos_seg, gout, arg, rt);                                \
    else if (pooled && lo)                                                                              \
      bwd_dma_kernel<KK, NN, NWV, OCC, true, true><<<grid, NWV * 64, 0, stream>>>(                      \
          gy, h, 0, 0, am, sc, bs, slope, c1, c2, c3, xprev, pam, psc, pbs, pslope, W, gx,         \
          gw_partial, pstat_partial, perm, pos_seg, gout, arg, rt);                                \
    else if (pooled)                                                                               \
      bwd_dma_kernel<KK, NN, NWV, OCC, false, true><<<grid, NWV * 64, 0, stream>>>(                     \
          gy, h, 0, 0, am, sc, bs, slope, c1, c2, c3, xprev, pam, psc, pbs, pslope, W, gx,         \
          gw_partial, pstat_partial, perm, pos_seg, gout, arg, rt);                                \
    else if (lo)                                                                                   \
      bwd_dma_kernel<KK, NN, NWV, OCC, true, false><<<grid, NWV * 64, 0, stream>>>(                     \
          gy, h, 0, 0, am, sc, bs, slope, c1, c2, c3, xprev, pam, psc, pbs, pslope, W, gx,         \
          gw_partial, pstat_partial, perm, pos_seg, gout, arg, rt);                                \
    else                                                                                           \
      bwd_dma_kernel<KK, NN, NWV, OCC, false, false><<<grid, NWV * 64, 0, stream>>>(                    \
          gy, h, 0, 0, am, sc, bs, slope, c1, c2, c3, xprev, pam, psc, pbs, pslope, W, gx,         \
          gw_partial, pstat_partial, perm, pos_seg, gout, arg, rt);                                \
    if (gw_tabs) *gw_tabs = (int)blocks;                                                           \
    return (int)blocks * NWV;                                                                      \
  }
  SPT_DMA_CASE(64, 128, 8, 1, 2)
  SPT_DMA_CASE(64, 64, 8, 1, 2)
  SPT_DMA_CASE(32, 64, 8, 2, 4)
#undef SPT_DMA_CASE
  return 0;
}

}
```

superpoint_transformer_amd/ops.py:

```python
import contextlib
import ctypes
import os

import torch

from . import _lib
from . import precision as _precision
from .csr import EdgeCSR, SegmentCSR, csr_of, edge_csr_of

_OPS = {"sum": 0, "add": 0, "mean": 1, "min": 2, "max": 3}

_TIMERS = {}
_TIMER_PREFIXES = []
_TIMER_CAP = 8192


def enable_timer(name, prefix=False):
    _TIMERS[name] = []
    if prefix and name not in _TIMER_PREFIXES:
        _TIMER_PREFIXES.append(name)


def timer_count(name):
    return len(_TIMERS.get(name) or [])
# ... 1497 lines not shown

    def c_arrays(self):
        if self._c is None:
            import ctypes
            n = self.n
            self._c = (n, (ctypes.c_int64 * n)(*self.r0), (ctypes.c_int64 * n)(*self.r1),
                       (ctypes.c_int32 * n)(*self.g))
        return self._c

    def rows_per_graph(self):
        out = [0] * self.B
        for a, b, g in zip(self.r0, self.r1, self.g):
            out[g] += b - a
        return out


def graph_runs(batch, num_graphs, rows):
    if batch is None or (num_graphs is not None and int(num_graphs) == 1):
        return GraphRuns([(0, rows, 0)], 1, rows)
    B = int(num_graphs)
    if B > MAX_FUSED_RUNS:
        return None
    memo = getattr(batch, _GRUN_ATTR, None)
    key = (batch._version, B, batch.data_ptr(), batch.numel())
    if memo is not None and memo[0] == key:
        return memo[1]
    runs = None
    hp = _host_ptr(batch, B)
    if batch.numel() == 0:
        runs = GraphRuns([], B, 0)
    elif hp is not None:
        runs = GraphRuns([(hp[g], hp[g + 1], g) for g in range(B) if hp[g + 1] > hp[g]], B,
                         batch.numel())
    else:
        change = (batch[1:] != batch[:-1])
        n_change = int(change.sum())
        if n_change + 1 <= MAX_FUSED_RUNS:
            starts = [0] + (torch.nonzero(change).flatten() + 1).tolist()
            ends = starts[1:] + [int(batch.numel())]
            ids = batch[torch.tensor(starts, device=batch.device)].tolist()
            if all(0 <= g < B for g in ids):
                runs = GraphRuns(list(zip(starts, ends, ids)), B, batch.numel())
    try:
        setattr(batch, _GRUN_ATTR, (key, runs))
    except Exception:
        pass
    return runs


_GRUN_ATTR = "_spt_graph_runs"


def graph_runs_via(batch, num_graphs, holder, *deps):
    key = tuple((d._version, d.data_ptr(), d.numel()) for d in deps) + (int(num_graphs),)
    memo = getattr(holder, _GRUN_ATTR + "_via", None)
    host = getattr(holder, "_spt_host_runs", None)
    if memo is not None and memo[0] == key:
        runs = memo[1]
    elif (host is not None and holder._version == 0 and host[0] == (int(num_graphs), batch.numel())
          and len(host[1]) <= MAX_FUSED_RUNS):
        runs = GraphRuns(list(host[1]), int(num_graphs), batch.numel())
    else:
        runs = graph_runs(batch, num_graphs, batch.numel())
        try:
            setattr(holder, _GRUN_ATTR + "_via", (key, runs))
        except Exception:
            pass
    try:
        setattr(batch, _GRUN_ATTR, ((batch._version, int(num_graphs), batch.data_ptr(), batch.numel()), runs))
    except Exception:
        pass
    return runs


def fused_mlp_supported(dims):
    return all(_lib.lib.spt_fused_linear_supported(int(k), int(n))
               for k, n in zip(dims[:-1], dims[1:]))


_ST_H, _ST_X = 8, 16


def _fmlp_forward(x, batch, runs, eps_list, slope_list, params, apply_last=True, fmode=-1,
                  store16=False):
    L = len(eps_list)
    Ws = [params[4 * i].detach().float().contiguous() for i in range(L)]
    gnw = [params[4 * i + 1].detach().float().contiguous() for i in range(L)]
    gnb = [params[4 * i + 2].detach().float().contiguous() for i in range(L)]
    gms = [params[4 * i + 3].detach().float().contiguous() for i in range(L)]
    x2 = x.detach().contiguous()
    if x2.dtype != torch.float32:
        x2 = x2.float()
    R = x2.shape[0]
    dev = x2.device
    B = runs.B
    nr, c_r0, c_r1, c_g = runs.c_arrays()
    sp = _lib.stream_ptr(dev)
    hs, tabs = [], []
    cur, pre = x2, None
    y = None
    with torch.cuda.device(dev):
        for l in range(L):
            N, K = Ws[l].shape
            h = torch.empty((R, N), dtype=torch.bfloat16 if store16 else torch.float32, device=dev)
            lmode = (3 | _ST_H | (_ST_X if l else 0)) if store16 else fmode
            total = torch.empty((B, 2 * N + 1), dtype=torch.float64, device=dev)
            nb = _lib.lib.spt_fused_linear_workspace_bytes(K, N)
            ws = _workspace(nb, dev)
            pa = ps = pb = None
            if pre is not None:
                pa, ps, pb = pre
            mean = torch.empty((B, N), dtype=torch.float32, device=dev)
            rstd, am, sc = (torch.empty_like(mean) for _ in range(3))
            if FUSE_POST:
                norm = _lib.GnFwdTables(_lib.ptr(gnw[l]), _lib.ptr(gms[l]), float(eps_list[l]),
                                        _lib.ptr(mean), _lib.ptr(rstd), _lib.ptr(am), _lib.ptr(sc))
                with _timed(f"fused_linear_fwd:{K}x{N}:{R}"):
                    st = _lib.lib.spt_fused_linear_fwd_runs_gn_f32(
                        _lib.ptr(cur), nr, c_r0, c_r1, c_g, B, K, _lib.ptr(Ws[l]), N,
                        _lib.ptr(pa), _lib.ptr(ps), _lib.ptr(pb),
                        float(slope_list[l - 1]) if l else 1.0, _lib.ptr(h),
                        _lib.ptr(total), lmode, _lib.ptr(ws), ws.numel(), ctypes.addressof(norm), sp)
                _lib.check(st, "spt_fused_linear_fwd_runs_gn_f32")
            else:
                with _timed(f"fused_linear_fwd:{K}x{N}:{R}"):
                    st = _lib.lib.spt_fused_linear_fwd_runs_f32(
                        _lib.ptr(cur), nr, c_r0, c_r1, c_g, B, K, _lib.ptr(Ws[l]), N,
                        _lib.ptr(pa), _lib.ptr(ps), _lib.ptr(pb),
                        float(slope_list[l - 1]) if l else 1.0, _lib.ptr(h),
                        _lib.ptr(total), lmode, _lib.ptr(ws), ws.numel(), sp)
                _lib.check(st, "spt_fused_linear_fwd_runs_f32")
                st = _lib.lib.spt_graphnorm_tables_f32(
                    _lib.ptr(total), B, N, _lib.ptr(gnw[l]), _lib.ptr(gms[l]), float(eps_list[l]),
                    _lib.ptr(mean), _lib.ptr(rstd), _lib.ptr(am), _lib.ptr(sc), sp)
                _lib.check(st, "spt_graphnorm_tables_f32")
            hs.append(h)
            tabs.append((mean, rstd, am, sc))
            cur, pre = h, (am, sc, gnb[l])
        if apply_last:
            assert not store16, "bf16 storage: the last norm is applied by the consumer (the pool)"
            N = Ws[-1].shape[0]
            y = torch.empty((R, N), dtype=torch.float32, device=dev)
            st = _lib.lib.spt_graphnorm_apply_f32(
                _lib.ptr(hs[-1]), _lib.ptr(batch) if B > 1 else None, R, N, B,
                _lib.ptr(tabs[-1][2]), _lib.ptr(tabs[-1][3]), _lib.ptr(gnb[-1]),
                float(slope_list[-1]), _lib.ptr(y), sp)
            _lib.check(st, "spt_graphnorm_apply_f32")
    saved = (x2, batch, *hs, *[t for tab in tabs for t in tab], *Ws, *gnw, *gnb, *gms)
    return y, saved, hs[-1], (tabs[-1][2], tabs[-1][3], gnb[-1])


FUSE_POST = os.environ.get("SPT_FUSE_POST", "1") != "0"


def fuse_post(on=None):
    global FUSE_POST
    old = FUSE_POST
    if on is not None:
        FUSE_POST = bool(on)
    return old


FOLD_BOTTOM = os.environ.get("SPT_FMLP_FOLD_BOTTOM", "1") != "0"


def fold_bottom(on=None):
    global FOLD_BOTTOM
    old = FOLD_BOTTOM
    if on is not None:
        FOLD_BOTTOM = bool(on)
    return old


def _fmlp_backward(saved, meta, gy, top_total=None, pooled=None, top_tabs=None):
    L, runs, slopes, in_dtype, need_gx0 = meta[:5]
    fmode = meta[5] if len(meta) > 5 else -1
    store16 = bool(meta[6]) if len(meta) > 6 else False
    sv = list(saved)
    x2, batch = sv[0], sv[1]
    hs = sv[2:2 + L]
    tabs = [tuple(sv[2 + L + 4 * i: 2 + L + 4 * i + 4]) for i in range(L)]
    o = 2 + 5 * L
    Ws, gnw, gnb, gms = sv[o:o + L], sv[o + L:o + 2 * L], sv[o + 2 * L:o + 3 * L], sv[o + 3 * L:o + 4 * L]
    R = x2.shape[0]
    dev = x2.device
    B = runs.B
    nr, c_r0, c_r1, c_g = runs.c_arrays()
    sp = _lib.stream_ptr(dev)
    g_cur = gy.contiguous().float() if gy is not None else None
    grads = [None] * (4 * L)
    gx0 = None
    with torch.cuda.device(dev):
        N = Ws[-1].shape[0]
        mean, rstd, am, sc = tabs[-1]
        if top_tabs is not None:
            total = None
        elif top_total is not None:
            total = top_total
        else:
            assert not store16, "bf16 storage: the top statistics come from the sparse route"
            total = torch.empty((B, 2 * N + 1), dtype=torch.float64, device=dev)
            ws = _workspace(_lib.lib.spt_graphnorm_workspace_bytes(R, N, B), dev)
            st = _lib.lib.spt_graphnorm_bwd_stats_f32(
                _lib.ptr(hs[-1]), _lib.ptr(g_cur), _lib.ptr(batch) if B > 1 else None, R, N, B,
                _lib.ptr(am), _lib.ptr(sc), _lib.ptr(gnb[-1]), float(slopes[-1]), _lib.ptr(total),
                _lib.ptr(ws), ws.numel(), sp)
            _lib.check(st, "spt_graphnorm_bwd_stats_f32")
        cur_tabs = top_tabs
        for l in range(L - 1, -1, -1):
            N, K = Ws[l].shape
            mean, rstd, am, sc = tabs[l]
            if cur_tabs is not None:
                c1, c2, c3, gw_n, gb_n, ga_n = cur_tabs
            else:
                c1, c2, c3 = (torch.empty((B, N), dtype=torch.float32, device=dev) for _ in range(3))
                gw_n, gb_n, ga_n = (torch.empty(N, dtype=torch.float32, device=dev) for _ in range(3))
                st = _lib.lib.spt_graphnorm_bwd_tables_f32(
                    _lib.ptr(total), B, N, _lib.ptr(gnw[l]), _lib.ptr(gms[l]), _lib.ptr(mean),
                    _lib.ptr(rstd), _lib.ptr(c1), _lib.ptr(c2), _lib.ptr(c3), _lib.ptr(gw_n),
                    _lib.ptr(gb_n), _lib.ptr(ga_n), sp)
                _lib.check(st, "spt_graphnorm_bwd_tables_f32")
            xprev = hs[l - 1] if l else x2
            pre = tabs[l - 1] if l else None
            lmode = (3 | _ST_H | (_ST_X if l else 0)) if store16 else fmode
            fold = (l == 1 and FOLD_BOTTOM and FUSE_POST and not need_gx0 and not store16
                    and not (pooled is not None and l == L - 1)
                    and x2.dtype == torch.float32 and x2.data_ptr() % 16 == 0
                    and bool(_lib.lib.spt_fused_linear_bwd_fold_supported(
                        int(Ws[0].shape[1]), K, N, lmode)))
            want_gx = (l > 0 or need_gx0) and not fold
            gx = torch.empty((R, K), dtype=torch.float32, device=dev) if want_gx else None
            gW = torch.empty((N, K), dtype=torch.float32, device=dev)
            nxt_tabs, pn = None, None
            if l and FUSE_POST:
                nxt_tabs = (*(torch.empty((B, K), dtype=torch.float32, device=dev) for _ in range(3)),
                            *(torch.empty(K, dtype=torch.float32, device=dev) for _ in range(3)))
                pn = _lib.GnBwdTables(_lib.ptr(gnw[l - 1]), _lib.ptr(gms[l - 1]), _lib.ptr(tabs[l - 1][0]),
                                      _lib.ptr(tabs[l - 1][1]), *[_lib.ptr(t) for t in nxt_tabs])
            ptot = (torch.empty((B, 2 * K + 1), dtype=torch.float64, device=dev)
                    if (l and pn is None) else None)
            ws = _workspace(_lib.lib.spt_fused_linear_workspace_bytes(K, N), dev)
            pa = ps = pb = None
            if pre is not None:
                pa, ps, pb = pre[2], pre[3], gnb[l - 1]
            if fold:
                K0 = int(Ws[0].shape[1])
                gW0 = torch.empty((K, K0), dtype=torch.float32, device=dev)
                with _timed(f"fused_linear_bwd_fold:{K0}x{K}x{N}:{R}"):
                    st = _lib.lib.spt_fused_linear_bwd_runs_gn_fold_f32(
                        _lib.ptr(g_cur), _lib.ptr(hs[l]), nr, c_r0, c_r1, c_g, B, N,
                        _lib.ptr(am), _lib.ptr(sc), _lib.ptr(gnb[l]), float(slopes[l]),
                        _lib.ptr(c1), _lib.ptr(c2), _lib.ptr(c3), _lib.ptr(xprev), K,
                        _lib.ptr(pa), _lib.ptr(ps), _lib.ptr(pb), float(slopes[0]), _lib.ptr(Ws[l]),
                        _lib.ptr(gW), lmode, _lib.ptr(ws), ws.numel(), ctypes.addressof(pn),
                        _lib.ptr(x2), K0, _lib.ptr(Ws[0]), _lib.ptr(gW0), sp)
                _lib.check(st, "spt_fused_linear_bwd_runs_gn_fold_f32")
                grads[4], grads[5], grads[6], grads[7] = gW, gw_n, gb_n, ga_n
                grads[0], grads[1], grads[2], grads[3] = gW0, nxt_tabs[3], nxt_tabs[4], nxt_tabs[5]
                break
            if pooled is not None and l == L - 1:
                p_gout, p_arg, p_csr = pooled
                args = (_lib.ptr(p_gout), _lib.ptr(p_arg), _lib.ptr(p_csr.perm),
                        _lib.ptr(p_csr.pos_seg()), _lib.ptr(hs[l]), nr, c_r0, c_r1, c_g, B, N,
                        _lib.ptr(am), _lib.ptr(sc), _lib.ptr(gnb[l]), float(slopes[l]),
                        _lib.ptr(c1), _lib.ptr(c2), _lib.ptr(c3), _lib.ptr(xprev), K,
                        _lib.ptr(pa), _lib.ptr(ps), _lib.ptr(pb),
                        float(slopes[l - 1]) if l else 1.0, _lib.ptr(Ws[l]), _lib.ptr(gx),
                        _lib.ptr(gW), _lib.ptr(ptot), lmode, _lib.ptr(ws), ws.numel())
                with _timed(f"fused_linear_bwd_pooled:{K}x{N}:{R}"):
                    if pn is not None:
                        st = _lib.lib.spt_fused_linear_bwd_pooled_runs_gn_f32(*args, ctypes.addressof(pn), sp)
                    else:
                        st = _lib.lib.spt_fused_linear_bwd_pooled_runs_f32(*args, sp)
                _lib.check(st, "spt_fused_linear_bwd_pooled_runs_f32")
            else:
                args = (_lib.ptr(g_cur), _lib.ptr(hs[l]), nr, c_r0, c_r1, c_g, B, N,
                        _lib.ptr(am), _lib.ptr(sc), _lib.ptr(gnb[l]), float(slopes[l]),
                        _lib.ptr(c1), _lib.ptr(c2), _lib.ptr(c3), _lib.ptr(xprev), K,
                        _lib.ptr(pa), _lib.ptr(ps), _lib.ptr(pb),
                        float(slopes[l - 1]) if l else 1.0, _lib.ptr(Ws[l]), _lib.ptr(gx),
                        _lib.ptr(gW), _lib.ptr(ptot), lmode, _lib.ptr(ws), ws.numel())
                if pn is not None:
                    st = _lib.lib.spt_fused_linear_bwd_runs_gn_f32(*args, ctypes.addressof(pn), sp)
                else:
                    st = _lib.lib.spt_fused_linear_bwd_runs_f32(*args, sp)
                _lib.check(st, "spt_fused_linear_bwd_runs_f32")
            grads[4 * l], grads[4 * l + 1], grads[4 * l + 2], grads[4 * l + 3] = gW, gw_n, gb_n, ga_n
            if l:
                g_cur, total, cur_tabs = gx, ptot, nxt_tabs
            else:
                gx0 = gx
    return (None if gx0 is None else gx0.to(in_dtype)), grads


class _FusedMLP(torch.autograd.Function):

    @staticmethod
    def forward(ctx, x, batch, runs, eps_list, slope_list, *params):
        fmode = _precision.fused_mode()
        y, saved, _, _ = _fmlp_forward(x, batch, runs, eps_list, slope_list, params, fmode=fmode)
        ctx.save_for_backward(*saved)
        ctx.meta = (len(eps_list), runs, list(slope_list), x.dtype, x.requires_grad, fmode)
        return y.to(x.dtype)

    @staticmethod
    def backward(ctx, gy):
        gx0, grads = _fmlp_backward(ctx.saved_tensors, ctx.meta, gy)
        return (gx0, None, None, None, None, *grads)


POOL_RAW_OUTPUT = True

POOL_IN_FORWARD = os.environ.get("SPT_POOL_IN_FORWARD", "1") != "0"


def pool_in_forward(on=None):
    global POOL_IN_FORWARD
    prev = POOL_IN_FORWARD
    if on is not None:
        POOL_IN_FORWARD = bool(on)
    return prev


class _FusedMLPMaxPool(torch.autograd.Function):

    @staticmethod
    def forward(ctx, x, batch, runs, eps_list, slope_list, csr, seg_graph, *params):
        fmode = _precision.fused_mode()
        L = len(eps_list)
        dims = [params[0].shape[1]] + [params[4 * i].shape[0] for i in range(L)]
        store16 = bool(
            _precision.bf16_activation_storage()
            and all(_lib.lib.spt_fused_linear_storage_supported(int(k), int(n))
                    for k, n in zip(dims[:-1], dims[1:]))
            and all(int(k) % 32 == 0 for k in dims[1:-1])
            and 256 % int(dims[-1]) == 0
            and _lib.lib.spt_segcsr_max_affine_bf16_supported(int(dims[-1]), x.shape[0]))
        ctx.pool_fused = False
        mode_top = (3 | _ST_X) if store16 else fmode
        if (POOL_IN_FORWARD and L > 1 and runs.sorted_batch
                and _lib.lib.spt_fused_linear_pool_supported(int(dims[-2]), int(dims[-1]), mode_top)
                and (runs.B == 1 or graph_ranges(seg_graph, runs.B, csr.num_seg) is not None)):
            return _FusedMLPMaxPool._forward_pooled(ctx, x, batch, runs, eps_list, slope_list, csr,
                                                    seg_graph, params, fmode, store16, mode_top)
        _, saved, h_last, (am, sc, bs) = _fmlp_forward(x, batch, runs, eps_list, slope_list,
                                                        params, apply_last=False, fmode=fmode,
                                                        store16=store16)
        R, N = h_last.shape
        dev = h_last.device
        out = torch.empty((csr.num_seg, N), dtype=torch.float32, device=dev)
        arg = torch.empty((csr.num_seg, N), dtype=torch.int32, device=dev)
        raw = None
        if (POOL_RAW_OUTPUT and any(ctx.needs_input_grad) and N <= 256 and 256 % N == 0
                and _lib.lib.spt_segcsr_max_affine_raw_supported(int(N), R)):
            raw = torch.empty((csr.num_seg, N), dtype=torch.float32, device=dev)
        with torch.cuda.device(dev), _timed(f"segcsr_reduce_fwd:3:{R}x{N}"):
            if raw is not None:
                st = _lib.lib.spt_segcsr_max_affine_raw_f32(
                    _lib.ptr(h_last), 1 if store16 else 0, _lib.ptr(csr.perm), _lib.ptr(csr.rowptr),
                    R, csr.num_seg, N, _lib.ptr(am), _lib.ptr(sc), _lib.ptr(bs),
                    float(slope_list[-1]), _lib.ptr(seg_graph), _lib.ptr(out), _lib.ptr(arg),
                    _lib.ptr(raw), _lib.stream_ptr(dev))
            else:
                seg_max = (_lib.lib.spt_segcsr_max_affine_bf16 if store16
                           else _lib.lib.spt_segcsr_max_affine_f32)
                st = seg_max(
                    _lib.ptr(h_last), _lib.ptr(csr.perm), _lib.ptr(csr.rowptr), R, csr.num_seg, N,
                    _lib.ptr(am), _lib.ptr(sc), _lib.ptr(bs), float(slope_list[-1]),
                    _lib.ptr(seg_graph), _lib.ptr(out), _lib.ptr(arg), _lib.stream_ptr(dev))
        _lib.check(st, "spt_segcsr_max_affine")
        ctx.has_raw = raw is not None
        if raw is not None:
            ctx.save_for_backward(arg, *saved, raw)
        else:
            ctx.save_for_backward(arg, *saved)
        ctx.csr = csr
        ctx.seg_graph = seg_graph
        ctx.meta = (len(eps_list), runs, list(slope_list), x.dtype, x.requires_grad,
                    3 if store16 else fmode, store16)
        return out.to(x.dtype)

    @staticmethod
    def _forward_pooled(ctx, x, batch, runs, eps_list, slope_list, csr, seg_graph, params, fmode,
                        store16, mode_top):
        L = len(eps_list)
        _, saved_sub, h_prev, (pam, psc, pbs) = _fmlp_forward(
            x, batch, runs, eps_list[:L - 1], slope_list[:L - 1], params[:4 * (L - 1)],
            apply_last=False, fmode=fmode, store16=store16)
        W = params[4 * (L - 1)].detach().float().contiguous()
        gnw, gnb, gms = (params[4 * (L - 1) + i].detach().float().contiguous() for i in (1, 2, 3))
        N, K = W.shape
        R = h_prev.shape[0]
        dev = h_prev.device
        B = runs.B
        S = csr.num_seg
        nr, c_r0, c_r1, c_g = runs.c_arrays()
        out = torch.empty((S, N), dtype=torch.float32, device=dev)
        arg = None
        argpos = torch.empty((S, N), dtype=torch.int32, device=dev)
        raw = torch.empty((S, N), dtype=torch.float32, device=dev)
        glen = int(_lib.lib.spt_fused_linear_pool_gram_len(K))
        gram = torch.empty((B, glen), dtype=torch.float64, device=dev)
        mean, rstd, am, sc = (torch.empty((B, N), dtype=torch.float32, device=dev) for _ in range(4))
        nb = _lib.lib.spt_fused_linear_pool_workspace_bytes(K, N)
        ws = _workspace(nb, dev)
        with torch.cuda.device(dev), _timed(f"fused_linear_fwd_pool:{K}x{N}:{R}"):
            st = _lib.lib.spt_fused_linear_fwd_pool_runs_f32(
                _lib.ptr(h_prev), _lib.ptr(csr.perm), _lib.ptr(csr.pos_seg()), _lib.ptr(csr.rowptr),
                _lib.ptr(seg_graph), S, R, nr, c_r0, c_r1, c_g, B, K, _lib.ptr(W), N,
                _lib.ptr(gnw), _lib.ptr(gnb), _lib.ptr(gms), float(eps_list[-1]),
                float(slope_list[-1]), _lib.ptr(pam), _lib.ptr(psc), _lib.ptr(pbs),
                float(slope_list[-2]), _lib.ptr(out), _lib.ptr(arg), _lib.ptr(argpos), _lib.ptr(raw),
                _lib.ptr(gram),
                None, _lib.ptr(mean), _lib.ptr(rstd), _lib.ptr(am), _lib.ptr(sc), mode_top,
                _lib.ptr(ws), ws.numel(), _lib.stream_ptr(dev))
        _lib.check(st, "spt_fused_linear_fwd_pool_runs_f32")
        ctx.pool_fused = True
        ctx.n_sub = len(saved_sub)
        ctx.save_for_backward(argpos, raw, gram, mean, rstd, am, sc, W, gnw, gnb, gms, h_prev, pam, psc,
                              pbs, argpos, *saved_sub)
        ctx.csr = csr
        ctx.seg_graph = seg_graph
        ctx.meta = (L, runs, list(slope_list), x.dtype, x.requires_grad,
                    3 if store16 else fmode, store16)
        ctx.mode_top = mode_top
        return out.to(x.dtype)

    @staticmethod
    def _backward_pooled(ctx, gout):
        (arg, raw, gram, mean, rstd, am, sc, W, gnw, gnb, gms, h_prev, pam, psc,
         pbs, argpos) = ctx.saved_tensors[:16]
        saved_sub = ctx.saved_tensors[16:]
        L, runs, slopes, in_dtype, need_gx0, fmode, store16 = ctx.meta
        N, K = W.shape
        R = h_prev.shape[0]
        dev = h_prev.device
        B = runs.B
        csr = ctx.csr
        S = csr.num_seg
        nr, c_r0, c_r1, c_g = runs.c_arrays()
        sp = _lib.stream_ptr(dev)
        gout = gout.contiguous().float()
        with torch.cuda.device(dev):
            total = torch.empty((B, 2 * N + 1), dtype=torch.float64, device=dev)
            rows = _const_tensor(runs.rows_per_graph(), torch.int64, dev)
            nbs = _lib.lib.spt_graphnorm_bwd_stats_sparse_workspace_bytes(S, N, B)
            ws = _workspace(nbs, dev)
            st = _lib.lib.spt_graphnorm_bwd_stats_sparse_raw_f32(
                _lib.ptr(raw), _lib.ptr(gout), _lib.ptr(arg), _lib.ptr(ctx.seg_graph),
                _lib.ptr(rows), S, R, N, B, _lib.ptr(am), _lib.ptr(sc), _lib.ptr(gnb),
                float(slopes[-1]), _lib.ptr(total), _lib.ptr(ws), nbs, sp)
            _lib.check(st, "spt_graphnorm_bwd_stats_sparse_raw_f32")
            c1, c2, c3 = (torch.empty((B, N), dtype=torch.float32, device=dev) for _ in range(3))
            gw_n, gb_n, ga_n = (torch.empty(N, dtype=torch.float32, device=dev) for _ in range(3))
            st = _lib.lib.spt_graphnorm_bwd_tables_f32(
                _lib.ptr(total), B, N, _lib.ptr(gnw), _lib.ptr(gms), _lib.ptr(mean), _lib.ptr(rstd),
                _lib.ptr(c1), _lib.ptr(c2), _lib.ptr(c3), _lib.ptr(gw_n), _lib.ptr(gb_n),
                _lib.ptr(ga_n), sp)
            _lib.check(st, "spt_graphnorm_bwd_tables_f32")
            gm = torch.empty((S, N), dtype=torch.float32, device=dev)
            gx = torch.empty((R, K), dtype=torch.float32, device=dev)
            gW = torch.empty((N, K), dtype=torch.float32, device=dev)
            Ls = L - 1
            sub_tabs, pn, ptot = None, None, None
            if FUSE_POST:
                o = 2 + 5 * Ls
                s_gnw, s_gms = saved_sub[o + Ls + Ls - 1], saved_sub[o + 3 * Ls + Ls - 1]
                s_mean, s_rstd = saved_sub[2 + Ls + 4 * (Ls - 1)], saved_sub[2 + Ls + 4 * (Ls - 1) + 1]
                sub_tabs = (*(torch.empty((B, K), dtype=torch.float32, device=dev) for _ in range(3)),
                            *(torch.empty(K, dtype=torch.float32, device=dev) for _ in range(3)))
                pn = _lib.GnBwdTables(_lib.ptr(s_gnw), _lib.ptr(s_gms), _lib.ptr(s_mean), _lib.ptr(s_rstd),
# ... 100 lines not shown
```

Measured before the change: 372.8.

## Recompute bottom MLP layer output inside next layer instead of storing it

Adds a rebuild route where the first fused linear layer (K0=12 -> 32) does not write its output to global memory. The second layer's forward kernel and the backward fold kernel recompute that output on the fly from the raw input x0 and W0 with split-bf16 MFMAs, applying the first layer's norm and activation inline. This removes the write and reread of the R x 32 intermediate in exchange for extra matrix work and LDS use. It is gated on no input gradient being needed, and on f32 non-storage mode with the DMA fold route.

```diff
diff --git a/include/spt_hip.h b/include/spt_hip.h
--- a/include/spt_hip.h
+++ b/include/spt_hip.h
@@ -568,6 +568,12 @@
     float pre_slope, const float* W, float* gx, float* gW, double* prev_total, int mode, void* ws,
     size_t ws_bytes, const spt_gn_bwd_tables* prev_norm, spt_stream_t stream);
 int spt_fused_linear_bwd_fold_supported(int K0, int K, int N, int mode);
+int spt_fused_linear_rebuild_supported(int K0, int K, int N, int mode);
+int spt_fused_linear_fwd_runs_gn_rebuild_f32(
+    const float* x0, int K0, const float* W0, int nruns, const int64_t* run_r0, const int64_t* run_r1,
+    const int32_t* run_graph, int num_graphs, int K, const float* W, int N, const float* pre_am,
+    const float* pre_scale, const float* pre_bias, float pre_slope, float* h, double* total, int mode,
+    void* ws, size_t ws_bytes, const spt_gn_fwd_tables* norm, spt_stream_t stream);
 int spt_fused_linear_bwd_runs_gn_fold_f32(
     const float* gy, const float* h, int nruns, const int64_t* run_r0, const int64_t* run_r1,
     const int32_t* run_graph, int num_graphs, int N, const float* am, const float* scale,
diff --git a/superpoint_transformer_amd/_lib.py b/superpoint_transformer_amd/_lib.py
--- a/superpoint_transformer_amd/_lib.py
+++ b/superpoint_transformer_amd/_lib.py
@@ -150,6 +150,10 @@
                                                 _p, _p, _p, _p, _int, _p, _p, _p, _f32, _p, _p, _p, _p,
                                                 _int, _p, _sz, _p, _p]),
     "spt_fused_linear_bwd_fold_supported": (_int, [_int, _int, _int, _int]),
+    "spt_fused_linear_rebuild_supported": (_int, [_int, _int, _int, _int]),
+    "spt_fused_linear_fwd_runs_gn_rebuild_f32": (_int, [_p, _int, _p, _int, _p, _p, _p, _int, _int, _p,
+                                                        _int, _p, _p, _p, _f32, _p, _p, _int, _p, _sz,
+                                                        _p, _p]),
     "spt_fused_linear_bwd_runs_gn_fold_f32": (_int, [_p, _p, _int, _p, _p, _p, _int, _int, _p, _p, _p, _f32,
                                                      _p, _p, _p, _p, _int, _p, _p, _p, _f32, _p, _p,
                                                      _int, _p, _sz, _p, _p, _int, _p, _p, _p]),
diff --git a/superpoint_transformer_amd/csrc/fused_mlp.hip b/superpoint_transformer_amd/csrc/fused_mlp.hip
--- a/superpoint_transformer_amd/csrc/fused_mlp.hip
+++ b/superpoint_transformer_amd/csrc/fused_mlp.hip
@@ -669,18 +669,24 @@
     l[i] = (__bf16)r2;
   }
 }
-template <int K4, int NBK>
-__global__ __launch_bounds__(WAVES_X3 * 64, 2) void fwd_kernel_x3(
+template <int K4, int NBK, int FK0>
+__device__ __forceinline__ void fwd_x3_body(
     const float* __restrict__ x, int64_t r0, int64_t r1, int K, const float* __restrict__ W,
     const float* __restrict__ am, const float* __restrict__ sc, const float* __restrict__ bs,
-    float slope, float* __restrict__ h, double* __restrict__ partial, FmlpRuns rt) {
+    float slope, float* __restrict__ h, double* __restrict__ partial, const FmlpRuns& rt,
+    const float* __restrict__ x0, const float* __restrict__ W0) {
   constexpr int KP = K4 * 4, KS = (KP + 31) / 32, KP32 = KS * 32, LDA = KP32 + 4, N = NBK * 16;
   constexpr int LDW = KP32 + 8;
+  constexpr bool RB = FK0 > 0;
+  static_assert(!RB || (KP == 32 && FK0 <= 32), "the rebuilt input is one 32-column k-step");
+  constexpr int LDW0 = 32 + 8;
   SPT_FMLP_RUN_FWD(N)
   __shared__ __attribute__((aligned(16))) float a_lds[WAVES_X3][TR * LDA];
   __shared__ __attribute__((aligned(16))) float tab[3 * KP32];
   __shared__ __attribute__((aligned(16))) __bf16 wpl[3][N * LDW];
   __shared__ double red[WAVES_X3][2 * N];
+  __shared__ __attribute__((aligned(16))) float x0_lds[RB ? WAVES_X3 : 1][RB ? TR * LDA : 4];
+  __shared__ __attribute__((aligned(16))) __bf16 w0pl[3][RB ? 32 * LDW0 : 8];
   const int lane = threadIdx.x & 63;
   const int wid = __builtin_amdgcn_readfirstlane(threadIdx.x >> 6);
   const int g = lane >> 4, c = lane & 15;
@@ -699,6 +705,19 @@
     wpl[1][n * LDW + k] = b[0];
     wpl[2][n * LDW + k] = cc[0];
   }
+  float* xl = x0_lds[RB ? wid : 0];
+  if constexpr (RB) {
+    for (int i = lane; i < TR * LDA; i += 64) xl[i] = 0.f;
+    for (int i = threadIdx.x; i < 32 * 32; i += WAVES_X3 * 64) {
+      const int n = i / 32, k = i - n * 32;
+      const float w1[1] = {(k < FK0) ? W0[(size_t)n * FK0 + k] : 0.f};
+      __bf16 a[1], b[1], cc[1];
+      split3_bf16<1>(w1, a, b, cc);
+      w0pl[0][n * LDW0 + k] = a[0];
+      w0pl[1][n * LDW0 + k] = b[0];
+      w0pl[2][n * LDW0 + k] = cc[0];
+    }
+  }
   __syncthreads();
 
   double s1[NBK], s2[NBK];
@@ -708,8 +727,23 @@
   const int64_t ntiles = (r1 - r0 + TR - 1) / TR;
   const int64_t wave = (int64_t)blockIdx.x * WAVES_X3 + wid;
   const int64_t nwaves = (int64_t)gridDim.x * WAVES_X3;
+  static_assert(FK0 % 4 == 0, "x0 rows of whole 16-byte chunks");
+  constexpr int NV0 = !RB ? 1 : (TR * FK0 / 4 + 63) / 64;
+  float4 pv0[NV0];
+  auto prefetch0 = [&](int64_t t) {
+    const int64_t row0 = r0 + t * TR;
+    const int cnt = (t < ntiles) ? (int)((r1 - row0) < TR ? (r1 - row0) : TR) : 0;
+    const float* xb = x0 + (cnt > 0 ? row0 : r0) * FK0;
+#pragma unroll
+    for (int j = 0; j < NV0; ++j) {
+      const int q = lane + 64 * j;
+      const bool ok = 4 * q < cnt * FK0;
+      const float4 v = *reinterpret_cast<const float4*>(xb + (ok ? 4 * q : 0));
+      pv0[j] = ok ? v : make_float4(0.f, 0.f, 0.f, 0.f);
+    }
+  };
   constexpr int CHP = KP / 4, NITP = (TR * CHP + 63) / 64;
-  const bool pref = (K & 3) == 0 && K == KP;
+  const bool pref = !RB && (K & 3) == 0 && K == KP;
   float4 pv[NITP];
   auto prefetch = [&](int64_t t) {
     const int64_t row0 = r0 + t * TR;
@@ -723,11 +757,54 @@
     }
   };
   if (pref && wave < ntiles) prefetch(wave);
+  if constexpr (RB) {
+    if (wave < ntiles) prefetch0(wave);
+  }
   for (int64_t t = wave; t < ntiles; t += nwaves) {
     const int64_t row0 = r0 + t * TR;
     const int cnt = (int)((r1 - row0) < TR ? (r1 - row0) : TR);
     wave_sync_lds();
-    if (pref) {
+    if constexpr (RB) {
+#pragma unroll
+      for (int j = 0; j < NV0; ++j) {
+        const int q = lane + 64 * j;
+        constexpr int CH0 = RB ? FK0 / 4 : 1;
+        const int rr = q / CH0, k = (q - rr * CH0) << 2;
+        if (q < TR * CH0) *reinterpret_cast<float4*>(xl + rr * LDA + k) = pv0[j];
+      }
+      wave_sync_lds();
+      prefetch0(t + nwaves);
+      const float4 b0 = *reinterpret_cast<const float4*>(xl + c * LDA + 8 * g);
+      const float4 b1 = *reinterpret_cast<const float4*>(xl + c * LDA + 8 * g + 4);
+      const float bv[8] = {b0.x, b0.y, b0.z, b0.w, b1.x, b1.y, b1.z, b1.w};
+      bf16x8 x1, x2, x3;
+      split3_bf16<8>(bv, x1, x2, x3);
+#pragma unroll
+      for (int nb = 0; nb < 2; ++nb) {
+        const int wo = (16 * nb + c) * LDW0 + 8 * g;
+        const bf16x8 w1 = *reinterpret_cast<const bf16x8*>(&w0pl[0][wo]);
+        const bf16x8 w2 = *reinterpret_cast<const bf16x8*>(&w0pl[1][wo]);
+        const bf16x8 w3 = *reinterpret_cast<const bf16x8*>(&w0pl[2][wo]);
+        f32x4 acc = (f32x4){0.f, 0.f, 0.f, 0.f};
+        acc = __builtin_amdgcn_mfma_f32_16x16x32_bf16(x3, w1, acc, 0, 0, 0);
+        acc = __builtin_amdgcn_mfma_f32_16x16x32_bf16(x1, w3, acc, 0, 0, 0);
+        acc = __builtin_amdgcn_mfma_f32_16x16x32_bf16(x2, w2, acc, 0, 0, 0);
+        acc = __builtin_amdgcn_mfma_f32_16x16x32_bf16(x2, w1, acc, 0, 0, 0);
+        acc = __builtin_amdgcn_mfma_f32_16x16x32_bf16(x1, w2, acc, 0, 0, 0);
+        acc = __builtin_amdgcn_mfma_f32_16x16x32_bf16(x1, w1, acc, 0, 0, 0);
+        const int col = 16 * nb + c;
+#pragma unroll
+        for (int r = 0; r < 4; ++r) {
+          const int rr = 4 * g + r;
+          float w = acc[r];
+          if (pre && rr < cnt) {
+            w = fmaf(w - tab[col], tab[KP32 + col], tab[2 * KP32 + col]);
+            w = w > 0.f ? w : w * slope;
+          }
+          al[rr * LDA + col] = w;
+        }
+      }
+    } else if (pref) {
 #pragma unroll
       for (int j = 0; j < NITP; ++j) {
         const int q = lane + 64 * j, rr = q / CHP, k = (q - rr * CHP) << 2;
@@ -780,11 +857,10 @@
     for (int r = 0; r < 4; ++r) {
       const int rr = 4 * g + r;
       if (rr < cnt) {
-        float* hr = h + (row0 + rr) * N + c;
 #pragma unroll
         for (int nb = 0; nb < NBK; ++nb) {
           const float v = C[nb][r];
-          hr[16 * nb] = v;
+          if (h) h[(row0 + rr) * N + c + 16 * nb] = v;
           s1[nb] += (double)v;
           s2[nb] += (double)v * (double)v;
         }
@@ -808,6 +884,23 @@
     out[i] = t2;
   }
   if (threadIdx.x == 0) out[2 * N] = (blockIdx.x == 0) ? (double)(r1 - r0) : 0.0;
+}
+
+template <int K4, int NBK>
+__global__ __launch_bounds__(WAVES_X3 * 64, 2) void fwd_kernel_x3(
+    const float* __restrict__ x, int64_t r0, int64_t r1, int K, const float* __restrict__ W,
+    const float* __restrict__ am, const float* __restrict__ sc, const float* __restrict__ bs,
+    float slope, float* __restrict__ h, double* __restrict__ partial, FmlpRuns rt) {
+  fwd_x3_body<K4, NBK, 0>(x, r0, r1, K, W, am, sc, bs, slope, h, partial, rt, nullptr, nullptr);
+}
+template <int K4, int NBK, int FK0>
+__global__ __launch_bounds__(WAVES_X3 * 64, 2) void fwd_kernel_x3_rb(
+    int64_t r0, int64_t r1, int K, const float* __restrict__ W, const float* __restrict__ am,
+    const float* __restrict__ sc, const float* __restrict__ bs, float slope, float* __restrict__ h,
+    double* __restrict__ partial, FmlpRuns rt, const float* __restrict__ x0,
+    const float* __restrict__ W0) {
+  static_assert(FK0 > 0, "the rebuilding instances");
+  fwd_x3_body<K4, NBK, FK0>(nullptr, r0, r1, K, W, am, sc, bs, slope, h, partial, rt, x0, W0);
 }
 
 __host__ __device__ constexpr bool fmlp_bf_wg_reduce(int K4, int NBK, int NW) {
@@ -1652,8 +1745,10 @@
                         const int32_t* pos_seg, const float* gout, const int32_t* arg,
                         hipStream_t stream, bool s16 = false, int* gw_tabs = nullptr,
                         const float* x0 = nullptr, const float* fshift = nullptr,
-                        float* fold_partial = nullptr, int K0 = 0, int blocks32 = 0);
+                        float* fold_partial = nullptr, int K0 = 0, int blocks32 = 0,
+                        const float* W0 = nullptr);
 bool fmlp_dma_fold_supported(int K0, int K, int N);
+bool fmlp_dma_rebuild_supported(int K0, int K, int N);
 bool fmlp_dma_dense_only(int K, int N);
 int fmlp_fold_len(int K, int K0);
 }
@@ -1756,12 +1851,21 @@
                          int num_graphs, int K, const float* W, int N, const float* pre_am,
                          const float* pre_scale, const float* pre_bias, float pre_slope, float* h,
                          double* total, int mode, void* ws, size_t ws_bytes, hipStream_t stream,
-                         const spt_gn_fwd_tables* norm = nullptr) {
+                         const spt_gn_fwd_tables* norm = nullptr, const float* x0 = nullptr,
+                         int K0 = 0, const float* W0 = nullptr) {
   const int g_fmlp_mode = fmlp_mode_of(mode);
   (void)fn;
   SPT_CHECK_ARG(K >= 1 && N >= 16, "bad shape");
   SPT_CHECK_ARG(spt_fused_linear_supported(K, N), "(K, N) not built");
-  SPT_CHECK_ARG(x && W && h && (total || norm) && ws, "null pointer");
+  SPT_CHECK_ARG((x || x0) && W && (total || norm) && ws, "null pointer");
+  const bool x3_route = g_fmlp_mode == 1 && g_fmlp_x3 &&
+                        !(mode >= 0 && (mode & (SPT_FMLP_H_BF16 | SPT_FMLP_X_BF16)));
+  SPT_CHECK_ARG(h || x3_route, "h == NULL: the default f32 mode's split forward only");
+  if (x0) {
+    SPT_CHECK_ARG(W0 && h && pre_am, "rebuild: W0, h and the bottom norm's tables");
+    SPT_CHECK_ARG(spt_fused_linear_rebuild_supported(K0, K, N, mode), "rebuild: shape pair or mode not built");
+    SPT_CHECK_ARG(((size_t)x0 & (K0 % 4 == 0 ? 15 : 3)) == 0, "rebuild: x0 alignment");
+  }
   SPT_CHECK_ARG(!norm || (norm->weight && norm->mean_scale && norm->mean && norm->rstd && norm->am &&
                           norm->scale), "incomplete norm tables");
   auto post = [&](const double* partial_, int gx__) {
@@ -1791,6 +1895,16 @@
   const dim3 grid((unsigned)gx_, (unsigned)rt.n);
   const dim3 grid8 = grid;
   double* partial = (double*)ws;
+  if (x0) {
+    if (K0 == 12 && k4 == 8 && nbk == 4)
+      fwd_kernel_x3_rb<8, 4, 12><<<grid8, WAVES_X3 * 64, 0, stream>>>(
+          0, 0, K, W, pre_am, pre_scale, pre_bias, pre_slope, h, partial, rt, x0, W0);
+    else
+      SPT_CHECK_ARG(false, "rebuild: no kernel for this shape pair");
+    post(partial, gx_);
+    SPT_CHECK_LAUNCH();
+    return 0;
+  }
   const bool h16 = mode >= 0 && (mode & SPT_FMLP_H_BF16), x16 = mode >= 0 && (mode & SPT_FMLP_X_BF16);
   if (h16 || x16) {
     SPT_CHECK_ARG(g_fmlp_mode == 3 && h16 && spt_fused_linear_storage_supported(K, N) &&
@@ -1880,6 +1994,26 @@
   SPT_CHECK_ARG(norm, "null norm descriptor");
   return fmlp_fwd_impl(__func__, x, rt, max_rows, num_graphs, K, W, N, pre_am, pre_scale, pre_bias,
                        pre_slope, h, total, mode, ws, ws_bytes, (hipStream_t)stream_, norm);
+}
+
+extern "C" int spt_fused_linear_rebuild_supported(int K0, int K, int N, int mode) {
+  const int m = fmlp_mode_of(mode);
+  if (mode >= 0 && (mode & (SPT_FMLP_H_BF16 | SPT_FMLP_X_BF16))) return 0;
+  return m == 1 && g_fmlp_x3 && fmlp_dma_of(mode) && fmlp_dma_rebuild_supported(K0, K, N) &&
+         spt_fused_linear_supported(K0, K);
+}
+extern "C" int spt_fused_linear_fwd_runs_gn_rebuild_f32(
+    const float* x0, int K0, const float* W0, int nruns, const int64_t* run_r0, const int64_t* run_r1,
+    const int32_t* run_graph, int num_graphs, int K, const float* W, int N, const float* pre_am,
+    const float* pre_scale, const float* pre_bias, float pre_slope, float* h, double* total, int mode,
+    void* ws, size_t ws_bytes, const spt_gn_fwd_tables* norm, spt_stream_t stream_) {
+  FmlpRuns rt;
+  int64_t max_rows;
+  const char* err = fmlp_make_runs(nruns, run_r0, run_r1, run_graph, num_graphs, &rt, &max_rows);
+  SPT_CHECK_ARG(!err, err ? err : "");
+  SPT_CHECK_ARG(norm && x0, "null pointer");
+  return fmlp_fwd_impl(__func__, nullptr, rt, max_rows, num_graphs, K, W, N, pre_am, pre_scale, pre_bias,
+                       pre_slope, h, total, mode, ws, ws_bytes, (hipStream_t)stream_, norm, x0, K0, W0);
 }
 
 static int fmlp_bwd_impl(bool pooled, const float* gy, const float* gout, const int32_t* arg,
@@ -1900,6 +2034,8 @@
                   "fold: dense layer, no gx, norm tables");
     SPT_CHECK_ARG(spt_fused_linear_bwd_fold_supported(fold_K0, K, N, mode), "fold: shape pair or mode not built");
     SPT_CHECK_ARG(((size_t)fold_x0 & (fold_K0 % 4 == 0 ? 15 : 3)) == 0, "fold: x0 alignment");
+    SPT_CHECK_ARG(xprev || spt_fused_linear_rebuild_supported(fold_K0, K, N, mode),
+                  "fold: xprev == NULL needs the rebuild route (shape pair, f32 mode, DMA-staged)");
   }
   const bool want_prev = prev_total || prev_norm;
   SPT_CHECK_ARG(!prev_norm || (prev_norm->weight && prev_norm->mean_scale && prev_norm->mean &&
@@ -1907,7 +2043,7 @@
                                prev_norm->gweight && prev_norm->gbias && prev_norm->gmean_scale),
                 "incomplete norm tables");
   SPT_CHECK_ARG(K >= 1 && N >= 16, "bad shape");
-  SPT_CHECK_ARG(h && am && scale && bias && c1 && c2 && c3 && xprev && W && gW && ws, "null pointer");
+  SPT_CHECK_ARG(h && am && scale && bias && c1 && c2 && c3 && (xprev || fold_x0) && W && gW && ws, "null pointer");
   SPT_CHECK_ARG(ws_bytes >= spt_fused_linear_workspace_bytes(K, N), "workspace too small");
   if (pooled) {
     SPT_CHECK_ARG(spt_fused_linear_pooled_supported_ex(K, N, g_fmlp_mode),
@@ -2080,7 +2216,7 @@
       per_run = fmlp_dma_bwd_launch(false, true, gy, h, rt, max_rows, N, am, scale, bias, slope, c1, c2,
                                     c3, xprev, K, pre_am, pre_scale, pre_bias, pre_slope, W, nullptr,
                                     gwp, pstp, nullptr, nullptr, nullptr, nullptr, stream, false,
-                                    &gw_tabs, fold_x0, fold_shift, fold_tabs, fold_K0, blocks32);
+                                    &gw_tabs, fold_x0, fold_shift, fold_tabs, fold_K0, blocks32, fold_W0);
     } else if (fold_K0 == 18 && k4 == 8 && nbk == 2) {
       constexpr int NWB = 4;
       gx_ = cap_grid(grid_for_nw(max_rows, 4, NWB), NWB);
diff --git a/superpoint_transformer_amd/csrc/fused_mlp_dma.hip b/superpoint_transformer_amd/csrc/fused_mlp_dma.hip
--- a/superpoint_transformer_amd/csrc/fused_mlp_dma.hip
+++ b/superpoint_transformer_amd/csrc/fused_mlp_dma.hip
@@ -93,8 +93,21 @@
 }
 
 constexpr int fold_len(int K, int K0) { return (K + (K0 + 16) / 16 * 16) * ((K0 + 16) / 16 * 16); }
-template <int K, int N, int NW, int OCC, bool LO, bool POOLED, bool S16 = false, int FK0 = 0>
-__global__ __launch_bounds__(NW * 64, OCC) void bwd_dma_kernel(
+template <int NV, typename V>
+__device__ __forceinline__ void split3_bf16(const float (&x)[NV], V& h, V& m, V& l) {
+#pragma unroll
+  for (int i = 0; i < NV; ++i) {
+    const __bf16 a = (__bf16)x[i];
+    const float r1 = x[i] - (float)a;
+    const __bf16 b = (__bf16)r1;
+    const float r2 = r1 - (float)b;
+    h[i] = a;
+    m[i] = b;
+    l[i] = (__bf16)r2;
+  }
+}
+template <int K, int N, int NW, int OCC, bool LO, bool POOLED, bool S16, int FK0, bool RB>
+__device__ __forceinline__ void bwd_dma_body(
     const float* __restrict__ gy, const float* __restrict__ h, int64_t r0, int64_t r1,
     const float* __restrict__ am, const float* __restrict__ sc, const float* __restrict__ bs,
     float slope, const float* __restrict__ c1, const float* __restrict__ c2,
@@ -103,10 +116,12 @@
     float pslope, const float* __restrict__ W, float* __restrict__ gx,
     float* __restrict__ gw_partial, double* __restrict__ pstat_partial,
     const int32_t* __restrict__ perm, const int32_t* __restrict__ pos_seg,
-    const float* __restrict__ gout, const int32_t* __restrict__ arg, FmlpRuns rt,
-    const float* __restrict__ x0 = nullptr, const float* __restrict__ fshift = nullptr,
-    float* __restrict__ fold_partial = nullptr) {
+    const float* __restrict__ gout, const int32_t* __restrict__ arg, const FmlpRuns& rt,
+    const float* __restrict__ x0, const float* __restrict__ fshift,
+    float* __restrict__ fold_partial, const float* __restrict__ W0) {
   constexpr bool FOLD = FK0 > 0;
+  static_assert(!RB || (FOLD && K == 32 && FK0 <= 32), "the rebuild rides on the fold's x0 tile");
+  constexpr int LDW0 = 32 + 8;
   constexpr int FOLD_K0 = FK0;
   static_assert(!FOLD || (!POOLED && !S16), "the fold reads dense f32 rows");
   constexpr int ZP = (FK0 + 16) / 16 * 16, ZB = ZP / 16;
@@ -141,6 +156,7 @@
   __shared__ __attribute__((aligned(16))) float pt[3 * K];
   __shared__ __attribute__((aligned(16))) float x0b[FOLD ? NW : 1][FOLD ? X0LEN : 4];
   __shared__ float fsh[32];
+  __shared__ __attribute__((aligned(16))) __bf16 w0pl[3][RB ? 32 * LDW0 : 8];
   const int lane = threadIdx.x & 63;
   const int wid = __builtin_amdgcn_readfirstlane(threadIdx.x >> 6);
   const int g = lane >> 4, c = lane & 15;
@@ -159,6 +175,17 @@
   if constexpr (FOLD) {
     if (threadIdx.x < 32) fsh[threadIdx.x] = threadIdx.x < FOLD_K0 ? fshift[threadIdx.x] : 0.f;
   }
+  if constexpr (RB) {
+    for (int i = threadIdx.x; i < 32 * 32; i += NW * 64) {
+      const int n = i / 32, k = i - n * 32;
+      const float w1[1] = {(k < FK0) ? W0[(size_t)n * FK0 + k] : 0.f};
+      __bf16 a[1], b[1], cc[1];
+      split3_bf16<1>(w1, a, b, cc);
+      w0pl[0][n * LDW0 + k] = a[0];
+      w0pl[1][n * LDW0 + k] = b[0];
+      w0pl[2][n * LDW0 + k] = cc[0];
+    }
+  }
   for (int i = threadIdx.x; i < K; i += NW * 64) {
     pt[i] = pre ? pam[i] : 0.f;
     pt[K + i] = pre ? psc[i] : 1.f;
@@ -293,7 +320,7 @@
       for (int i = 0; i < XI16; ++i)
         lds_dma16(xb + (int64_t)pick_lane<RX16>(rid_l, RX16 * i, x16) * K + 8 * q16,
                   XB + W_X / 2 + 256 * i);
-    } else {
+    } else if constexpr (!RB) {
       const float* xb = POOLED ? xprev : xprev + row0 * K;
       const int hx = ln / KC, px = ln % KC;
 #pragma unroll
@@ -382,6 +409,36 @@
         }
       }
     }
+    if constexpr (RB) {
+      static_assert(FK0 % 2 == 0, "x0 rows of whole 8-byte pairs");
+      float bv[8];
+#pragma unroll
+      for (int j = 0; j < 4; ++j) {
+        const bool ok = 8 * g + 2 * j < FOLD_K0 && c < cnt;
+        const float2 v = *reinterpret_cast<const float2*>(X0B + (ok ? c * FOLD_K0 + 8 * g + 2 * j : 0));
+        bv[2 * j] = ok ? v.x : 0.f;
+        bv[2 * j + 1] = ok ? v.y : 0.f;
+      }
+      bf16x8 x1, x2, x3;
+      split3_bf16<8>(bv, x1, x2, x3);
+#pragma unroll
+      for (int nb = 0; nb < KB; ++nb) {
+        const int wo = (16 * nb + c) * LDW0 + 8 * g;
+        const bf16x8 w1 = *reinterpret_cast<const bf16x8*>(&w0pl[0][wo]);
+        const bf16x8 w2 = *reinterpret_cast<const bf16x8*>(&w0pl[1][wo]);
+        const bf16x8 w3 = *reinterpret_cast<const bf16x8*>(&w0pl[2][wo]);
+        f32x4 acc = (f32x4){0.f, 0.f, 0.f, 0.f};
+        acc = __builtin_amdgcn_mfma_f32_16x16x32_bf16(x3, w1, acc, 0, 0, 0);
+        acc = __builtin_amdgcn_mfma_f32_16x16x32_bf16(x1, w3, acc, 0, 0, 0);
+        acc = __builtin_amdgcn_mfma_f32_16x16x32_bf16(x2, w2, acc, 0, 0, 0);
+        acc = __builtin_amdgcn_mfma_f32_16x16x32_bf16(x2, w1, acc, 0, 0, 0);
+        acc = __builtin_amdgcn_mfma_f32_16x16x32_bf16(x1, w2, acc, 0, 0, 0);
+        acc = __builtin_amdgcn_mfma_f32_16x16x32_bf16(x1, w1, acc, 0, 0, 0);
+#pragma unroll
+        for (int r = 0; r < 4; ++r)
+          XB[(4 * g + r) * K + 4 * ((4 * nb + (c >> 2)) ^ (4 * (g & 1))) + (c & 3)] = acc[r];
+      }
+    }
     lds_order();
     if constexpr (!(SPT_FDMA_SKIP & 2)) {
       bf16x4 Xh[KB], Xl[KB];
@@ -595,11 +652,44 @@
   }
 }
 
+template <int K, int N, int NW, int OCC, bool LO, bool POOLED, bool S16 = false, int FK0 = 0>
+__global__ __launch_bounds__(NW * 64, OCC) void bwd_dma_kernel(
+    const float* __restrict__ gy, const float* __restrict__ h, int64_t r0, int64_t r1,
+    const float* __restrict__ am, const float* __restrict__ sc, const float* __restrict__ bs,
+    float slope, const float* __restrict__ c1, const float* __restrict__ c2,
+    const float* __restrict__ c3, const float* __restrict__ xprev,
+    const float* __restrict__ pam, const float* __restrict__ psc, const float* __restrict__ pbs,
+    float pslope, const float* __restrict__ W, float* __restrict__ gx,
+    float* __restrict__ gw_partial, double* __restrict__ pstat_partial,
+    const int32_t* __restrict__ perm, const int32_t* __restrict__ pos_seg,
+    const float* __restrict__ gout, const int32_t* __restrict__ arg, FmlpRuns rt,
+    const float* __restrict__ x0 = nullptr, const float* __restrict__ fshift = nullptr,
+    float* __restrict__ fold_partial = nullptr) {
+  bwd_dma_body<K, N, NW, OCC, LO, POOLED, S16, FK0, false>(
+      gy, h, r0, r1, am, sc, bs, slope, c1, c2, c3, xprev, pam, psc, pbs, pslope, W, gx, gw_partial,
+      pstat_partial, perm, pos_seg, gout, arg, rt, x0, fshift, fold_partial, nullptr);
+}
+template <int K, int N, int NW, int OCC, int FK0>
+__global__ __launch_bounds__(NW * 64, OCC) void bwd_dma_kernel_rb(
+    const float* __restrict__ gy, const float* __restrict__ h, int64_t r0, int64_t r1,
+    const float* __restrict__ am, const float* __restrict__ sc, const float* __restrict__ bs,
+    float slope, const float* __restrict__ c1, const float* __restrict__ c2,
+    const float* __restrict__ c3, const float* __restrict__ pam, const float* __restrict__ psc,
+    const float* __restrict__ pbs, float pslope, const float* __restrict__ W,
+    float* __restrict__ gw_partial, double* __restrict__ pstat_partial, FmlpRuns rt,
+    const float* __restrict__ x0, const float* __restrict__ fshift,
+    float* __restrict__ fold_partial, const float* __restrict__ W0) {
+  bwd_dma_body<K, N, NW, OCC, true, false, false, FK0, true>(
+      gy, h, r0, r1, am, sc, bs, slope, c1, c2, c3, nullptr, pam, psc, pbs, pslope, W, nullptr,
+      gw_partial, pstat_partial, nullptr, nullptr, nullptr, nullptr, rt, x0, fshift, fold_partial, W0);
+}
+
 }
 
 bool fmlp_dma_fold_supported(int K0, int K, int N) {
   return (K0 == 12 && K == 32 && N == 64) || (K0 == 18 && K == 32 && N == 32);
 }
+bool fmlp_dma_rebuild_supported(int K0, int K, int N) { return K0 == 12 && K == 32 && N == 64; }
 int fmlp_fold_len(int K, int K0) { return fdma::fold_len(K, K0); }
 bool fmlp_dma_supported(int K, int N) {
   return (K == 64 && N == 128) || (K == 32 && N == 64) || (K == 64 && N == 64) || (K == 32 && N == 32);
@@ -615,7 +705,8 @@
                         float* gw_partial, double* pstat_partial, const int32_t* perm,
                         const int32_t* pos_seg, const float* gout, const int32_t* arg,
                         hipStream_t stream, bool s16, int* gw_tabs, const float* x0,
-                        const float* fshift, float* fold_partial, int K0, int blocks32) {
+                        const float* fshift, float* fold_partial, int K0, int blocks32,
+                        const float* W0) {
   using namespace fdma;
   const int64_t tiles = (max_rows + TR - 1) / TR;
   const int nr = rt.n < 1 ? 1 : rt.n;
@@ -624,6 +715,7 @@
     const dim3 grid((unsigned)blocks32, (unsigned)nr);
     if (x0) {
       if (!fmlp_dma_fold_supported(K0, K, N) || !lo || !fshift || !fold_partial || !pam) return 0;
+      if (!xprev) return 0;
       bwd_dma_kernel<32, 32, 4, 4, true, false, false, 18><<<grid, 4 * 64, 0, stream>>>(
           gy, h, 0, 0, am, sc, bs, slope, c1, c2, c3, xprev, pam, psc, pbs, pslope, W, nullptr,
           gw_partial, pstat_partial, perm, pos_seg, gout, arg, rt, x0, fshift, fold_partial);
@@ -646,6 +738,12 @@
     if (blocks > cap) blocks = cap;
     if (blocks < 1) blocks = 1;
     const dim3 grid((unsigned)blocks, (unsigned)nr);
+    if (!xprev) {
+      if (!W0) return 0;
+      bwd_dma_kernel_rb<32, 64, 8, 4, 12><<<grid, 8 * 64, 0, stream>>>(
+          gy, h, 0, 0, am, sc, bs, slope, c1, c2, c3, pam, psc, pbs, pslope, W, gw_partial,
+          pstat_partial, rt, x0, fshift, fold_partial, W0);
+    } else
     bwd_dma_kernel<32, 64, 8, 4, true, false, false, 12><<<grid, 8 * 64, 0, stream>>>(
         gy, h, 0, 0, am, sc, bs, slope, c1, c2, c3, xprev, pam, psc, pbs, pslope, W, nullptr,
         gw_partial, pstat_partial, perm, pos_seg, gout, arg, rt, x0, fshift, fold_partial);
diff --git a/superpoint_transformer_amd/ops.py b/superpoint_transformer_amd/ops.py
--- a/superpoint_transformer_amd/ops.py
+++ b/superpoint_transformer_amd/ops.py
@@ -1603,7 +1603,7 @@
 
 
 def _fmlp_forward(x, batch, runs, eps_list, slope_list, params, apply_last=True, fmode=-1,
-                  store16=False):
+                  store16=False, need_gx0=True):
     L = len(eps_list)
     Ws = [params[4 * i].detach().float().contiguous() for i in range(L)]
     gnw = [params[4 * i + 1].detach().float().contiguous() for i in range(L)]
@@ -1620,10 +1620,15 @@
     hs, tabs = [], []
     cur, pre = x2, None
     y = None
+    rebuild = (L >= 2 and x.dtype == torch.float32 and x2.data_ptr() % 16 == 0
+               and fused_mlp_rebuild_route(int(Ws[0].shape[1]), int(Ws[1].shape[1]),
+                                           int(Ws[1].shape[0]), fmode, need_gx0, store16))
     with torch.cuda.device(dev):
         for l in range(L):
             N, K = Ws[l].shape
-            h = torch.empty((R, N), dtype=torch.bfloat16 if store16 else torch.float32, device=dev)
+            h = None
+            if not (rebuild and l == 0):
+                h = torch.empty((R, N), dtype=torch.bfloat16 if store16 else torch.float32, device=dev)
             lmode = (3 | _ST_H | (_ST_X if l else 0)) if store16 else fmode
             total = torch.empty((B, 2 * N + 1), dtype=torch.float64, device=dev)
             nb = _lib.lib.spt_fused_linear_workspace_bytes(K, N)
@@ -1633,7 +1638,17 @@
                 pa, ps, pb = pre
             mean = torch.empty((B, N), dtype=torch.float32, device=dev)
             rstd, am, sc = (torch.empty_like(mean) for _ in range(3))
-            if FUSE_POST:
+            if rebuild and l == 1:
+                K0 = int(Ws[0].shape[1])
+                norm = _lib.GnFwdTables(_lib.ptr(gnw[l]), _lib.ptr(gms[l]), float(eps_list[l]),
+                                        _lib.ptr(mean), _lib.ptr(rstd), _lib.ptr(am), _lib.ptr(sc))
+                with _timed(f"fused_linear_fwd_rebuild:{K0}x{K}x{N}:{R}"):
+                    st = _lib.lib.spt_fused_linear_fwd_runs_gn_rebuild_f32(
+                        _lib.ptr(x2), K0, _lib.ptr(Ws[0]), nr, c_r0, c_r1, c_g, B, K, _lib.ptr(Ws[l]), N,
+                        _lib.ptr(pa), _lib.ptr(ps), _lib.ptr(pb), float(slope_list[0]), _lib.ptr(h),
+                        _lib.ptr(total), lmode, _lib.ptr(ws), ws.numel(), ctypes.addressof(norm), sp)
+                _lib.check(st, "spt_fused_linear_fwd_runs_gn_rebuild_f32")
+            elif FUSE_POST:
                 norm = _lib.GnFwdTables(_lib.ptr(gnw[l]), _lib.ptr(gms[l]), float(eps_list[l]),
                                         _lib.ptr(mean), _lib.ptr(rstd), _lib.ptr(am), _lib.ptr(sc))
                 with _timed(f"fused_linear_fwd:{K}x{N}:{R}"):
@@ -1691,6 +1706,27 @@
     if on is not None:
         FOLD_BOTTOM = bool(on)
     return old
+
+
+def _rebuild_default(environ):
+    return environ.get("SPT_FMLP_REBUILD_BOTTOM", "1") != "0"
+
+
+REBUILD_BOTTOM = _rebuild_default(os.environ)
+
+
+def rebuild_bottom(on=None):
+    global REBUILD_BOTTOM
+    old = REBUILD_BOTTOM
+    if on is not None:
+        REBUILD_BOTTOM = bool(on)
+    return old
+
+
+def fused_mlp_rebuild_route(K0, K, N, fmode=-1, need_gx0=False, store16=False):
+    return bool(REBUILD_BOTTOM and FOLD_BOTTOM and FUSE_POST and not need_gx0 and not store16
+                and _lib.lib.spt_fused_linear_bwd_fold_supported(int(K0), int(K), int(N), fmode)
+                and _lib.lib.spt_fused_linear_rebuild_supported(int(K0), int(K), int(N), fmode))
 
 
 def _fmlp_backward(saved, meta, gy, top_total=None, pooled=None, top_tabs=None):
@@ -1749,6 +1785,9 @@
                     and x2.dtype == torch.float32 and x2.data_ptr() % 16 == 0
                     and bool(_lib.lib.spt_fused_linear_bwd_fold_supported(
                         int(Ws[0].shape[1]), K, N, lmode)))
+            if l == 1 and xprev is None and not fold:
+                raise RuntimeError("the forward ran the rebuild route (no stored bottom output) but the "
+                                   "backward cannot take the fold: a switch changed in between")
             want_gx = (l > 0 or need_gx0) and not fold
             gx = torch.empty((R, K), dtype=torch.float32, device=dev) if want_gx else None
             gW = torch.empty((N, K), dtype=torch.float32, device=dev)
@@ -1819,7 +1858,8 @@
     @staticmethod
     def forward(ctx, x, batch, runs, eps_list, slope_list, *params):
         fmode = _precision.fused_mode()
-        y, saved, _, _ = _fmlp_forward(x, batch, runs, eps_list, slope_list, params, fmode=fmode)
+        y, saved, _, _ = _fmlp_forward(x, batch, runs, eps_list, slope_list, params, fmode=fmode,
+                                       need_gx0=x.requires_grad)
         ctx.save_for_backward(*saved)
         ctx.meta = (len(eps_list), runs, list(slope_list), x.dtype, x.requires_grad, fmode)
         return y.to(x.dtype)
@@ -1866,7 +1906,8 @@
                                                     seg_graph, params, fmode, store16, mode_top)
         _, saved, h_last, (am, sc, bs) = _fmlp_forward(x, batch, runs, eps_list, slope_list,
                                                         params, apply_last=False, fmode=fmode,
-                                                        store16=store16)
+                                                        store16=store16,
+                                                        need_gx0=x.requires_grad or L < 3)
         R, N = h_last.shape
         dev = h_last.device
         out = torch.empty((csr.num_seg, N), dtype=torch.float32, device=dev)
@@ -1907,7 +1948,7 @@
         L = len(eps_list)
         _, saved_sub, h_prev, (pam, psc, pbs) = _fmlp_forward(
             x, batch, runs, eps_list[:L - 1], slope_list[:L - 1], params[:4 * (L - 1)],
-            apply_last=False, fmode=fmode, store16=store16)
+            apply_last=False, fmode=fmode, store16=store16, need_gx0=x.requires_grad)
         W = params[4 * (L - 1)].detach().float().contiguous()
         gnw, gnb, gms = (params[4 * (L - 1) + i].detach().float().contiguous() for i in (1, 2, 3))
         N, K = W.shape
```

Result: no change. 375.1, median of 6 (+0.6%).
